# simonamtoft/downsampled-diffusion

Measured on AMD Instinct MI355X. Metric: images/sec (T=1000 sampling), 256x256 dDDPM-x3, higher is better.
Workload: dtype f32

## Files before the change

### downsampled-diffusion_amd/csrc/conv_igemm.hip

```cpp
#include <cstdlib>

#include "conv_common.h"

namespace ddk {

struct IgemmParams {
    const float* src0;
    const float* src1;
    const float* w;
    const float* bias;
    const float* resid;
    float* out;
    int c0, c1, cin;
    int B, H, W;
    int Hm, Wm;
    int Ho, Wo;
    int N, M;
    int in_stride, out_scale;
    int ntaps, nphase;
    int splits, kiters, kiters_per_split;
    long long slab_stride;
    int pre_mish, post_mish;
    float* mish_out;
    const float* dmish_src;
// ... 1093 lines not shown

int conv_init_device() {
#define HALO_ATTR(V) DDK_TRY(allow_lds(&conv3x3_halo_kernel<V>, (size_t)HALO_LDS_FLOATS * sizeof(float)));
    DDK_HALO_VARIANTS(HALO_ATTR)
#undef HALO_ATTR
#define C32_ATTR(WW)                                                                                      \
    DDK_TRY(allow_lds(&conv3x3_c32_kernel<WW, false>, (size_t)C32_LDS_BYTES));          \
    DDK_TRY(allow_lds(&conv3x3_c32_kernel<WW, true>, (size_t)C32_LDS_BYTES));
    DDK_C32_WIDTHS(C32_ATTR)
#undef C32_ATTR
#define DMA_ATTR(BM, BN, WM, WN, NS) DDK_TRY(allow_lds(&igemm_dma_kernel<BM, BN, WM, WN, NS>, dma_lds_bytes<BM, BN, WM, WN, NS>()));
    DMA_ATTR(128, 128, 2, 2, 2)
    DMA_ATTR(128, 64, 2, 2, 2) DMA_ATTR(128, 64, 2, 2, 4)
    DMA_ATTR(64, 64, 2, 2, 2) DMA_ATTR(64, 64, 2, 2, 4) DMA_ATTR(64, 64, 2, 2, 6)
    DMA_ATTR(128, 32, 4, 1, 2)
    DMA_ATTR(64, 32, 2, 1, 2)
#undef DMA_ATTR
    DDK_TRY(allow_lds(&igemm_kernel<128, 128, 2, 2>, reg_lds_bytes(128, 128)));
    DDK_TRY(allow_lds(&igemm_kernel<128, 64, 2, 2>, reg_lds_bytes(128, 64)));
    DDK_TRY(allow_lds(&igemm_kernel<64, 64, 2, 2>, reg_lds_bytes(64, 64)));
    DDK_TRY(allow_lds(&igemm_kernel<128, 32, 4, 1>, reg_lds_bytes(128, 32)));
    DDK_TRY(allow_lds(&igemm_kernel<64, 32, 2, 1>, reg_lds_bytes(64, 32)));
    return DDK_OK;
}

size_t conv_workspace_bytes(int kind, int B, int H, int W, int cin, int N) {
    Geometry g;
    if (!conv_geometry(kind, H, W, g) || cin <= 0 || cin % 32) return 0;
    const Choice c = plan_conv(kind, B, H, W, cin, N, g).c;
    size_t need = c.splits == 1 ? 0 : (size_t)c.splits * B * g.Ho * g.Wo * N * sizeof(float);
    if (kind == DDK_CONVT4X4_S2 && convT_wino_ok(H, W, cin, N)) {
        const int s = convT_wino_splits(B, H, W, cin, N);
        const size_t w = s == 1 ? 0 : (size_t)s * B * g.Ho * g.Wo * N * sizeof(float);
        if (w > need) need = w;
    }
    return need;
}

bool conv_ln_fold_ok(int B, int H, int W, int cin, int N) {
    const bool off = tuning_flag("DDK_NO_LN_FOLD");
    Geometry g;
    if (off || !conv_geometry(DDK_CONV1X1, H, W, g) || cin <= 0 || cin % 32 || N % 32) return false;
    const Choice c = choose_tile((long long)B * H * W, N, 1, cin / 32);
    return c.splits == 1 && (c.tile == T64x64 || c.tile == T128x64 || c.tile == T128x128);
}

int conv_forward(const ddk_conv_args& a, hipStream_t st, const ConvLnFold* ln, const WinoGnFuse* fuse) {
    Geometry g;
    DDK_REQUIRE(conv_geometry(a.kind, a.H, a.W, g), "conv kind");
    DDK_REQUIRE(a.src0 && a.out, "conv: null src0/out");
    DDK_REQUIRE(a.weight || a.weight_wino, "conv: null weight");
    DDK_REQUIRE(a.c0 > 0 && a.c0 % 32 == 0, "conv: c0 must be a positive multiple of 32");
    DDK_REQUIRE((a.src1 == nullptr) == (a.c1 == 0), "conv: src1/c1 mismatch");
    DDK_REQUIRE(a.c1 % 32 == 0, "conv: c1 must be a multiple of 32");
    DDK_REQUIRE(a.N > 0 && a.N % 32 == 0, "conv: N must be a positive multiple of 32");
    DDK_REQUIRE(a.B > 0 && a.H > 0 && a.W > 0, "conv: B/H/W");
    DDK_REQUIRE(aligned16(a.src0) && aligned16(a.src1) && aligned16(a.weight) && aligned16(a.out) &&
                    aligned16(a.bias) && aligned16(a.resid),
                "conv: pointers must be 16-byte aligned");
    DDK_REQUIRE((long long)a.B * g.Ho * g.Wo * a.N < (1LL << 31) && (long long)a.B * a.H * a.W * (a.c0 + a.c1) < (1LL << 31),
                "conv: tensor too large for 32-bit pixel indexing");

#ifdef DDK_HOST_SANITIZE
    {
        const long long pix_in = (long long)a.B * a.H * a.W, pix_out = (long long)a.B * g.Ho * g.Wo;
        san::extent("conv src0", a.src0, pix_in * a.c0 * 4);
        san::extent("conv src1", a.src1, pix_in * a.c1 * 4);
        if (!a.defer_reduce) san::extent("conv out", a.out, pix_out * a.N * 4);
        san::extent("conv resid", a.resid, pix_out * a.N * 4);
        san::extent("conv bias", a.bias, (long long)a.N * 4);
        san::extent("conv workspace", a.workspace, (long long)a.workspace_bytes);
        san::extent("conv mish_out", a.mish_out, pix_out * a.N * 4);
        san::extent("conv dmish_src", a.dmish_src, pix_out * a.N * 4);
        if (a.gn_partials && a.gn_groups > 0) san::extent("conv gn_partials", a.gn_partials, (pix_out / 128) * a.gn_groups * 8);
    }
#endif
    DDK_REQUIRE(aligned16(a.mish_out) && aligned16(a.dmish_src), "conv: mish_out / dmish_src alignment");
    DDK_REQUIRE(!(a.mish_out || a.dmish_src) || !(a.defer_reduce || a.gn_partials || fuse || ln),
                "conv: mish_out / dmish_src go with a plain conv (no deferred reduce, GroupNorm partials or LayerNorm folding)");
    const bool act_epilogue = a.mish_out || a.dmish_src;
    if (a.weight_wino && !a.pre_mish && !act_epilogue && conv_wino_ok(a.kind, a.H, a.W, a.c0 + a.c1, a.N)) {
        DDK_REQUIRE(aligned16(a.weight_wino), "conv: weight_wino alignment");
        DDK_TRY(ensure_device_init());
        const int ws = conv_wino_splits(a.B, a.H, a.W, a.c0 + a.c1, a.N);
        const long long slab = (long long)a.B * a.H * a.W * a.N;
        if (ws > 1) {
            const size_t need = (size_t)(fuse ? ws - 1 : ws) * slab * sizeof(float);
            if (!a.workspace || a.workspace_bytes < need) {
                set_error("conv(wino): split-K workspace too small (%zu < %zu)", a.workspace_bytes, need);
                return DDK_ERR_WORKSPACE;
            }
            DDK_REQUIRE(aligned16(a.workspace), "conv: workspace alignment");
        }
        DDK_REQUIRE((long long)a.B * a.H * a.W * (a.c0 > a.c1 ? a.c0 : a.c1) * 4 < (1LL << 31), "conv(wino): a source of 2 GiB or more");
        DDK_TRY(conv_wino_forward(a, ws, st, fuse));
        if (ws > 1 && !a.defer_reduce && !fuse) {
            const long long n4 = slab / 4;
            const int blocks = (int)(ceil_div(n4, 256) < 2048 ? ceil_div(n4, 256) : 2048);
            hipLaunchKernelGGL(splitk_reduce_kernel, dim3(blocks), dim3(256), 0, st, static_cast<const float*>(a.workspace), ws, slab, a.bias,
                               a.resid, a.out, n4, a.N, a.post_mish, static_cast<float*>(nullptr), static_cast<const float*>(nullptr));
            DDK_TRY(check_launch("splitk_reduce_kernel"));
        }
        return DDK_OK;
    }
    if (a.kind == DDK_CONVT4X4_S2 && a.weight_wino && a.c1 == 0 && !a.pre_mish && !a.post_mish && !a.resid && !act_epilogue && !a.gn_partials &&
        !fuse && !ln && convT_wino_ok(a.H, a.W, a.c0, a.N)) {
        DDK_REQUIRE(aligned16(a.weight_wino), "conv: weight_wino alignment");
        DDK_TRY(ensure_device_init());
        const int ws = convT_wino_splits(a.B, a.H, a.W, a.c0, a.N);
        const long long slab = (long long)a.B * g.Ho * g.Wo * a.N;
        if (ws > 1) {
            const size_t need = (size_t)(fuse ? ws - 1 : ws) * slab * sizeof(float);
            if (!a.workspace || a.workspace_bytes < need) {
                set_error("conv(winoT): split-K workspace too small (%zu < %zu)", a.workspace_bytes, need);
                return DDK_ERR_WORKSPACE;
            }
            DDK_REQUIRE(aligned16(a.workspace), "conv: workspace alignment");
        }
        DDK_REQUIRE((long long)a.B * a.H * a.W * a.c0 * 4 < (1LL << 31), "conv(winoT): a source of 2 GiB or more");
        DDK_TRY(convT_wino_forward(a, ws, st));
        if (ws > 1 && !a.defer_reduce && !fuse) {
            const long long n4 = slab / 4;
            const int blocks = (int)(ceil_div(n4, 256) < 2048 ? ceil_div(n4, 256) : 2048);
            hipLaunchKernelGGL(splitk_reduce_kernel, dim3(blocks), dim3(256), 0, st, static_cast<const float*>(a.workspace), ws, slab, a.bias,
                               a.resid, a.out, n4, a.N, a.post_mish, static_cast<float*>(nullptr), static_cast<const float*>(nullptr));
            DDK_TRY(check_launch("splitk_reduce_kernel"));
        }
        return DDK_OK;
    }
    DDK_REQUIRE(a.weight, "conv: weight is null and the shape / arguments do not take the Winograd path (ddk_conv_wino_splits() == 0, "
                          "pre_mish, mish_out or dmish_src)");
    if (a.kind == DDK_CONV1X1 && a.c1 == 0 && !a.pre_mish && !a.post_mish && !a.defer_reduce && !a.gn_partials && !fuse && !act_epilogue &&
        !tuning_flag("DDK_NO_CONV1X1_WS") && conv1x1_ws_ok((long long)a.B * a.H * a.W, a.c0, a.N) &&
        ((long long)a.B * a.H * a.W / 64) * (a.N / 128) >= 256 &&
        (!ln || ((long long)a.B * a.H * a.W / 64) * (a.N / 128) >= 16 * 256 ||
         (256 % (a.N / 128) == 0 && ((long long)a.B * a.H * a.W / 64) % (256 / (a.N / 128)) == 0))) {
        return conv1x1_ws(a.src0, a.weight, a.bias, a.resid, a.out, (long long)a.B * a.H * a.W, a.N, ln, st);
    }
    if (a.kind == DDK_CONV1X1 && !a.pre_mish && !a.post_mish && !a.defer_reduce && !a.gn_partials && !fuse && !act_epilogue &&
        !tuning_flag("DDK_NO_CONV1X1_SM") && conv1x1_sm_ok((long long)a.B * a.H * a.W, a.c0, a.c1, a.N) &&
        (!ln || (a.c1 == 0 && ((long long)a.B * a.H * a.W / 32) * (a.N / 32) <= 512)))
        return conv1x1_sm(a.src0, a.c0, a.src1, a.c1, a.weight, a.bias, a.resid, a.out, (long long)a.B * a.H * a.W, a.N, ln, st);
    if (a.kind == DDK_CONV1X1 && a.c1 == 0 && !a.defer_reduce && !a.gn_partials && !fuse && !ln && !tuning_flag("DDK_NO_CONV1X1_STREAM") &&
        conv1x1_stream_ok((long long)a.B * a.H * a.W, a.c0, a.N))
        return conv1x1_stream(a.src0, a.c0, a.weight, a.bias, a.dmish_src, a.resid, a.out, a.mish_out, (long long)a.B * a.H * a.W, a.N,
                              a.pre_mish, a.post_mish, st);
    DDK_REQUIRE(!a.gn_partials, "conv: gn_partials is only produced by the Winograd path (weight_wino given, ddk_conv_gn_partials() > 0)");
    DDK_REQUIRE(!fuse, "conv: the in-launch GroupNorm exists on the Winograd path only");
    IgemmParams p{};
    p.src0 = a.src0; p.src1 = a.src1; p.w = a.weight; p.bias = a.bias; p.resid = a.resid; p.out = a.out;
    p.c0 = a.c0; p.c1 = a.c1; p.cin = a.c0 + a.c1;
    p.B = a.B; p.H = a.H; p.W = a.W;
    p.Hm = g.Hm; p.Wm = g.Wm; p.Ho = g.Ho; p.Wo = g.Wo;
    p.N = a.N; p.M = a.B * g.Hm * g.Wm;
    p.in_stride = g.in_stride; p.out_scale = g.out_scale;
    p.ntaps = g.ntaps; p.nphase = g.nphase;
    p.kiters = g.ntaps * (p.cin / 32);
    p.pre_mish = a.pre_mish;
    p.debug = tuning_int("DDK_DEBUG", 0);
    p.post_mish = a.post_mish;
    p.mish_out = a.mish_out; p.dmish_src = a.dmish_src;
    p.slab_stride = (long long)a.B * g.Ho * g.Wo * a.N;
    p.dWm = make_fastdiv_u((unsigned)g.Wm);
    p.dHm = make_fastdiv_u((unsigned)g.Hm);
    p.tapmode = (a.kind == DDK_CONV1X1) ? 0 : (a.kind == DDK_CONVT4X4_S2 ? 2 : (a.kind == DDK_CONV4X4_S2 ? 3 : 1));
    if (!ln && !a.defer_reduce && choose_c32(a.kind, a.B, a.H, a.W, p.cin, p.N, a.c1, a.pre_mish != 0)) {
        const int TR = 128 / a.W, TB = TR > a.H ? TR / a.H : 1, rows_img = TB > 1 ? a.H : TR;
// ... 92 lines not shown
```

### downsampled-diffusion_amd/csrc/conv_wino.hip

```cpp
#include <atomic>
#include <cstdlib>
#include <type_traits>
#include <utility>

#include "cluster_sync.h"
#include "conv_common.h"
#include "pack_elems.h"

namespace ddk {

__device__ __attribute__((aligned(128))) float g_wino_zero[32];

struct WinoParams {
    const float* src0;
    const float* src1;
    const float* wu;
    const float* bias;
    const float* resid;
    float* out;
    int c0, c1, cin;
    int B, H, W, TH, TW;
    int N, tiles;
    int splits, chunks, chunks_per_split;
    long long slab_stride;
// ... 483 lines not shown
    const long long mt = ceil_div((long long)B * (H / 2) * (W / 2), WBT);
    return (N % 128 == 0 && mt * (N / 128) >= 224) ? WINO_V_F : WINO_V_D;
}
static int wino_nt(int variant) { return variant == WINO_V_F ? 128 : WBN; }
bool conv_wino_ok(int kind, int H, int W, int cin, int N) {
    return kind == DDK_CONV3X3_S1 && H >= 2 && W >= 2 && H % 2 == 0 && W % 2 == 0 && cin > 0 && cin % 32 == 0 && N % 64 == 0;
}

int conv_wino_splits(int B, int H, int W, int cin, int N) {
    const long long tiles = (long long)B * (H / 2) * (W / 2);
    const long long wgs = ceil_div(tiles, WBT) * (N / wino_nt(wino_variant(B, H, W, N)));
    const int chunks = cin / 32;
    int s = 1;
    while (wgs * s < 256 && s * 2 <= chunks) s *= 2;
    const int cps = (int)ceil_div(chunks, s);
    return (int)ceil_div(chunks, cps);
}

static int wino_stats_shape_parts(int B, int H, int W, int cin, int N, int groups) {
    if (!conv_wino_ok(DDK_CONV3X3_S1, H, W, cin, N) || groups <= 0 || N % groups) return 0;
    const int cpg = N / groups, tpi = (H / 2) * (W / 2), nt_w = wino_nt(wino_variant(B, H, W, N));
    if (cpg % 4 || nt_w % cpg || nt_w / cpg > 8 || tpi % WBT || tpi / WBT > 32) return 0;
    return tpi / WBT;
}
int conv_wino_stats_parts(int B, int H, int W, int cin, int N, int groups) {
    if (conv_wino_splits(B, H, W, cin, N) != 1) return 0;
    return wino_stats_shape_parts(B, H, W, cin, N, groups);
}

bool convT_wino_ok(int H, int W, int cin, int N) {
    return H >= 2 && W >= 2 && H % 2 == 0 && W % 2 == 0 && cin > 0 && cin % 32 == 0 && N > 0 && N % WT_NT == 0;
}
int convT_wino_splits(int B, int H, int W, int cin, int N) {
    const long long wgs = ceil_div((long long)B * (H / 2) * (W / 2), WBT) * (N / WT_NT) * 4;
    const int chunks = cin / 32;
    int s = 1;
    while (wgs * s < 256 && s * 2 <= chunks) s *= 2;
    const int cps = (int)ceil_div(chunks, s);
    return (int)ceil_div(chunks, cps);
}
int convT_wino_forward(const ddk_conv_args& a, int splits, hipStream_t st) {
    WinoParams p{};
    p.src0 = a.src0; p.wu = a.weight_wino; p.bias = a.bias; p.out = a.out;
    p.c0 = a.c0; p.c1 = 0; p.cin = a.c0;
    p.B = a.B; p.H = a.H; p.W = a.W; p.TH = a.H / 2; p.TW = a.W / 2;
    p.N = a.N; p.tiles = a.B * p.TH * p.TW;
    p.chunks = p.cin / 32;
    p.chunks_per_split = (int)ceil_div(p.chunks, splits);
    p.splits = (int)ceil_div(p.chunks, p.chunks_per_split);
    p.slab_stride = (long long)a.B * (2 * a.H) * (2 * a.W) * a.N;
    p.dTW = make_fastdiv_u((unsigned)p.TW);
    p.dTH = make_fastdiv_u((unsigned)p.TH);
    if (p.splits > 1) p.out = static_cast<float*>(a.workspace);
    dim3 grid((unsigned)ceil_div(p.tiles, WBT), (unsigned)(a.N / WT_NT), (unsigned)(4 * p.splits));
#ifdef DDK_TUNING
    if (getenv("DDK_WINO_STAMPS")) {
        hipLaunchKernelGGL(convT_wino_kernel<1>, grid, dim3(1024), WT_LDS_FL * sizeof(float), st, p);
        return check_launch("convT_wino_kernel<dbg>");
    }
#endif
    hipLaunchKernelGGL(convT_wino_kernel<0>, grid, dim3(1024), WT_LDS_FL * sizeof(float), st, p);
    return check_launch("convT_wino_kernel");
}

int conv_wino_init_device() {
    DDK_HIP(hipFuncSetAttribute(reinterpret_cast<const void*>(&convT_wino_kernel<0>), hipFuncAttributeMaxDynamicSharedMemorySize,
                                (int)(WT_LDS_FL * sizeof(float))));
#ifdef DDK_TUNING
    DDK_HIP(hipFuncSetAttribute(reinterpret_cast<const void*>(&convT_wino_kernel<1>), hipFuncAttributeMaxDynamicSharedMemorySize,
                                (int)(WT_LDS_FL * sizeof(float))));
#endif
    DDK_HIP(hipFuncSetAttribute(reinterpret_cast<const void*>(&conv3x3_wino_kernel<0>), hipFuncAttributeMaxDynamicSharedMemorySize,
                                (int)(W_LDS_FLOATS * sizeof(float))));
    DDK_HIP(hipFuncSetAttribute(reinterpret_cast<const void*>(&conv3x3_wino_kernel<0, true>), hipFuncAttributeMaxDynamicSharedMemorySize,
                                (int)(W_LDS_FLOATS * sizeof(float))));
    DDK_HIP(hipFuncSetAttribute(reinterpret_cast<const void*>(&conv3x3_wino2_kernel<2, 0, false>), hipFuncAttributeMaxDynamicSharedMemorySize,
                                (int)(W2<2>::LDS_FL * sizeof(float))));
    DDK_HIP(hipFuncSetAttribute(reinterpret_cast<const void*>(&conv3x3_wino2_kernel<2, 0, true>), hipFuncAttributeMaxDynamicSharedMemorySize,
                                (int)(W2<2>::LDS_FL * sizeof(float))));
    DDK_HIP(hipFuncSetAttribute(reinterpret_cast<const void*>(&conv3x3_wino2_kernel<4, 0, false>), hipFuncAttributeMaxDynamicSharedMemorySize,
                                (int)(W2<4>::LDS_FL * sizeof(float))));
    DDK_HIP(hipFuncSetAttribute(reinterpret_cast<const void*>(&conv3x3_wino2_kernel<4, 0, true>), hipFuncAttributeMaxDynamicSharedMemorySize,
                                (int)(W2<4>::LDS_FL * sizeof(float))));
#ifdef DDK_TUNING
#define W2_DBG_ATTR(P_, D_) DDK_HIP(hipFuncSetAttribute(reinterpret_cast<const void*>(&conv3x3_wino2_kernel<P_, D_, false>), \
                                                hipFuncAttributeMaxDynamicSharedMemorySize, (int)(W2<P_>::LDS_FL * sizeof(float))))
    W2_DBG_ATTR(2, 1); W2_DBG_ATTR(2, 7); W2_DBG_ATTR(2, 9); W2_DBG_ATTR(2, 15); W2_DBG_ATTR(2, 17);
    W2_DBG_ATTR(4, 1); W2_DBG_ATTR(4, 7); W2_DBG_ATTR(4, 9); W2_DBG_ATTR(4, 15); W2_DBG_ATTR(4, 17);
#undef W2_DBG_ATTR
    DDK_HIP(hipFuncSetAttribute(reinterpret_cast<const void*>(&conv3x3_wino_kernel<1>), hipFuncAttributeMaxDynamicSharedMemorySize, (int)(W_LDS_FLOATS * sizeof(float))));
    DDK_HIP(hipFuncSetAttribute(reinterpret_cast<const void*>(&conv3x3_wino_kernel<2>), hipFuncAttributeMaxDynamicSharedMemorySize, (int)(W_LDS_FLOATS * sizeof(float))));
    DDK_HIP(hipFuncSetAttribute(reinterpret_cast<const void*>(&conv3x3_wino_kernel<3>), hipFuncAttributeMaxDynamicSharedMemorySize, (int)(W_LDS_FLOATS * sizeof(float))));
    DDK_HIP(hipFuncSetAttribute(reinterpret_cast<const void*>(&conv3x3_wino_kernel<4>), hipFuncAttributeMaxDynamicSharedMemorySize, (int)(W_LDS_FLOATS * sizeof(float))));
#endif
    return DDK_OK;
}

int conv_wino_cluster_np(int B, int H, int W, int cin, int N, int groups) {
    const int np = conv_wino_stats_parts(B, H, W, cin, N, groups);
    if (np <= 0 || np > 8) return 0;
    const int nt_w = wino_nt(wino_variant(B, H, W, N));
    if (N / groups > 32 || nt_w % (N / groups)) return 0;
    if (nt_w / (N / groups) > 8) return 0;
    const long long mt = (long long)B * np, nt = N / nt_w;
    if ((mt * nt) % 8) return 0;
    const long long run = mt * nt / 8;
    const long long per_round = run < 32 ? run : 32;
    if (run % (np * nt) || per_round % (np * nt)) return 0;
    return np;
}
int conv_wino_cluster_split_np(int B, int H, int W, int cin, int N, int groups, int* splits_out) {
    if (!conv_wino_ok(DDK_CONV3X3_S1, H, W, cin, N)) return 0;
    const int splits = conv_wino_splits(B, H, W, cin, N);
    if (splits_out) *splits_out = splits;
    if (splits <= 1 || splits > 4) return 0;
    const int np = wino_stats_shape_parts(B, H, W, cin, N, groups);
    if (np <= 0 || np > 8) return 0;
    const int variant = wino_variant(B, H, W, N);
    if (variant != WINO_V_D) return 0;
    const int nt_w = wino_nt(variant);
    if (N / groups > 32 || nt_w % (N / groups) || nt_w / (N / groups) > 8) return 0;
    const long long mt = (long long)B * np, nt = N / nt_w;
    if (mt * nt * splits > 256) return 0;
    return np;
}
size_t conv_wino_cluster_pair_words(int B, int H, int W, int N) {
    return (size_t)ceil_div((long long)B * (H / 2) * (W / 2), WBT) * (size_t)(N / WBN) * 16;
}
size_t conv_wino_cluster_ws_floats(int B, int H, int W, int N) {
    const long long mt = (long long)B * (H / 2) * (W / 2) / WBT, nt = N / WBN;
    return (size_t)(mt * nt * 32 + (long long)B * nt * 16);
}

bool conv_wino_cluster_device_ok() {
    static std::atomic<int> cached[64];
    int dev = 0;
    if (hipGetDevice(&dev) != hipSuccess || dev < 0 || dev >= 64) return false;
    int v = cached[dev].load(std::memory_order_relaxed);
    if (v == 0) {
        int cus = 0, xccs = 0;
        bool ok = hipDeviceGetAttribute(&cus, hipDeviceAttributeMultiprocessorCount, dev) == hipSuccess && cus == 256;
        ok = ok && hipDeviceGetAttribute(&xccs, hipDeviceAttributeNumberOfXccs, dev) == hipSuccess && xccs == 8;
        ok = ok && !getenv("HSA_CU_MASK") && !getenv("ROC_GLOBAL_CU_MASK");
        (void)hipGetLastError();
        v = ok ? 1 : 2;
        cached[dev].store(v, std::memory_order_relaxed);
    }
    return v == 1;
}

bool conv_wino_variant_new(int B, int H, int W, int N) { return wino_variant(B, H, W, N) != WINO_V_OLD; }

int conv_wino_forward(const ddk_conv_args& a, int splits, hipStream_t st, const WinoGnFuse* fuse) {
    WinoParams p{};
    if (fuse) {
        const int np = splits == 1 ? conv_wino_cluster_np(a.B, a.H, a.W, a.c0 + a.c1, a.N, fuse->groups)
                                   : conv_wino_cluster_split_np(a.B, a.H, a.W, a.c0 + a.c1, a.N, fuse->groups, nullptr);
        DDK_REQUIRE(np > 0 && !a.post_mish && !a.gn_partials, "conv(wino): shape not eligible for the in-launch GroupNorm");
        if (splits > 1) {
            DDK_REQUIRE(fuse->pairs && a.workspace && aligned16(a.workspace) && !fuse->res_x,
                        "conv(wino, cluster): a split shape needs pair counters and the slab workspace");
            p.cl_slab = static_cast<float*>(a.workspace);
            p.cl_pair = fuse->pairs;
        }
        DDK_REQUIRE(fuse->gamma && fuse->beta && fuse->records && fuse->counters && aligned16(fuse->gamma) && aligned16(fuse->beta) &&
                        aligned16(fuse->temb) && fuse->temb_stride % 4 == 0 && aligned16(fuse->records) && aligned16(fuse->counters),
                    "conv(wino): in-launch GroupNorm arguments");
        p.gn_gamma = fuse->gamma; p.gn_beta = fuse->beta; p.gn_temb = fuse->temb; p.gn_temb_rows = fuse->temb_rows;
        p.gn_temb_stride = fuse->temb_stride; p.gn_eps = fuse->eps;
        p.cl_rec = fuse->records; p.cl_cnt = fuse->counters; p.cl_fail = fuse->fail; p.cl_np = np;
        if (fuse->res_x) {
            DDK_REQUIRE(fuse->res_w && fuse->res_cin > 0 && fuse->res_cin <= 8 && fuse->res_ld >= fuse->res_cin && !a.resid,
                        "conv(wino, cluster): the 1x1 addend takes <= 8 input channels and excludes a tensor addend");
            DDK_REQUIRE(wino_variant(a.B, a.H, a.W, a.N) != WINO_V_OLD, "conv(wino, cluster): the 1x1 addend exists in the 8-matrix-wave kernels only");
            p.r1_x = fuse->res_x; p.r1_w = fuse->res_w; p.r1_b = fuse->res_b; p.r1_cin = fuse->res_cin; p.r1_ld = fuse->res_ld;
        }
        p.groups = fuse->groups;
        p.cpg = a.N / fuse->groups;
    }
    if (a.gn_partials) {
        DDK_REQUIRE(conv_wino_stats_parts(a.B, a.H, a.W, a.c0 + a.c1, a.N, a.gn_groups) > 0 && splits == 1 && !a.resid && !a.post_mish,
                    "conv: gn_partials needs a shape with ddk_conv_gn_partials() > 0 and no resid / post_mish");
        DDK_REQUIRE((reinterpret_cast<uintptr_t>(a.gn_partials) & 7u) == 0, "conv: gn_partials alignment");
        p.gn_part = reinterpret_cast<float2*>(a.gn_partials);
        p.groups = a.gn_groups;
        p.cpg = a.N / a.gn_groups;
    }
    p.src0 = a.src0; p.src1 = a.src1; p.wu = a.weight_wino; p.bias = a.bias; p.resid = a.resid; p.out = a.out;
    p.c0 = a.c0; p.c1 = a.c1; p.cin = a.c0 + a.c1;
    p.B = a.B; p.H = a.H; p.W = a.W; p.TH = a.H / 2; p.TW = a.W / 2;
    p.N = a.N; p.tiles = a.B * p.TH * p.TW;
    p.chunks = p.cin / 32;
    p.chunks_per_split = (int)ceil_div(p.chunks, splits);
    p.splits = (int)ceil_div(p.chunks, p.chunks_per_split);
    p.slab_stride = (long long)a.B * a.H * a.W * a.N;
    p.post_mish = a.post_mish;
    p.dTW = make_fastdiv_u((unsigned)p.TW);
    p.dTH = make_fastdiv_u((unsigned)p.TH);
    if (p.splits > 1 && !fuse) p.out = static_cast<float*>(a.workspace);
    const int variant = wino_variant(a.B, a.H, a.W, a.N);
    if (variant != WINO_V_OLD) {
        dim3 grid2((unsigned)ceil_div(p.tiles, WBT), (unsigned)(a.N / wino_nt(variant)), (unsigned)p.splits);
        const bool f = variant == WINO_V_F;
        const size_t lds = (size_t)(f ? W2<2>::LDS_FL : W2<4>::LDS_FL) * sizeof(float);
#ifdef DDK_TUNING
        if (getenv("DDK_WINO_STAMPS")) {
            const int v = getenv("DDK_WINO_DEBUG") ? atoi(getenv("DDK_WINO_DEBUG")) : 1;
#define W2_DBG_LAUNCH(D_)                                                                                              \
    if (v == D_) {                                                                                                     \
        if (f) hipLaunchKernelGGL((conv3x3_wino2_kernel<2, D_, false>), grid2, dim3(768), lds, st, p);                 \
        else hipLaunchKernelGGL((conv3x3_wino2_kernel<4, D_, false>), grid2, dim3(768), lds, st, p);                   \
        return check_launch("conv3x3_wino2_kernel<dbg>");                                                              \
    }
            W2_DBG_LAUNCH(7) W2_DBG_LAUNCH(9) W2_DBG_LAUNCH(15) W2_DBG_LAUNCH(17)
#undef W2_DBG_LAUNCH
            if (f) hipLaunchKernelGGL((conv3x3_wino2_kernel<2, 1, false>), grid2, dim3(768), lds, st, p);
            else hipLaunchKernelGGL((conv3x3_wino2_kernel<4, 1, false>), grid2, dim3(768), lds, st, p);
            return check_launch("conv3x3_wino2_kernel<dbg>");
        }
#endif
        if (fuse) {
            if (f) hipLaunchKernelGGL((conv3x3_wino2_kernel<2, 0, true>), grid2, dim3(768), lds, st, p);
            else hipLaunchKernelGGL((conv3x3_wino2_kernel<4, 0, true>), grid2, dim3(768), lds, st, p);
            return check_launch("conv3x3_wino2_kernel<cluster>");
        }
        if (f) hipLaunchKernelGGL((conv3x3_wino2_kernel<2, 0, false>), grid2, dim3(768), lds, st, p);
        else hipLaunchKernelGGL((conv3x3_wino2_kernel<4, 0, false>), grid2, dim3(768), lds, st, p);
        return check_launch("conv3x3_wino2_kernel");
    }
    dim3 grid((unsigned)ceil_div(p.tiles, WBT), (unsigned)(a.N / WBN), (unsigned)p.splits);
#ifdef DDK_TUNING
    if (getenv("DDK_WINO_STAMPS")) {
        const int v = getenv("DDK_WINO_DEBUG") ? atoi(getenv("DDK_WINO_DEBUG")) : 1;
        if (v == 2) hipLaunchKernelGGL(conv3x3_wino_kernel<2>, grid, dim3(512), W_LDS_FLOATS * sizeof(float), st, p);
        else if (v == 3) hipLaunchKernelGGL(conv3x3_wino_kernel<3>, grid, dim3(512), W_LDS_FLOATS * sizeof(float), st, p);
        else if (v == 4) hipLaunchKernelGGL(conv3x3_wino_kernel<4>, grid, dim3(512), W_LDS_FLOATS * sizeof(float), st, p);
        else hipLaunchKernelGGL(conv3x3_wino_kernel<1>, grid, dim3(512), W_LDS_FLOATS * sizeof(float), st, p);
        return check_launch("conv3x3_wino_kernel<dbg>");
    }
#endif
    if (fuse) {
        hipLaunchKernelGGL((conv3x3_wino_kernel<0, true>), grid, dim3(512), W_LDS_FLOATS * sizeof(float), st, p);
        return check_launch("conv3x3_wino_kernel<cluster>");
    }
    hipLaunchKernelGGL(conv3x3_wino_kernel<0>, grid, dim3(512), W_LDS_FLOATS * sizeof(float), st, p);
    return check_launch("conv3x3_wino_kernel");
}

__global__ __launch_bounds__(256) void occupy_kernel(unsigned long long ticks, unsigned* sink) {
    extern __shared__ float occupy_lds[];
    occupy_lds[threadIdx.x] = (float)threadIdx.x;
    __syncthreads();
    const unsigned long long t_begin = __builtin_amdgcn_s_memrealtime();
    while (__builtin_amdgcn_s_memrealtime() - t_begin < ticks) __builtin_amdgcn_s_sleep(32);
    if (occupy_lds[(threadIdx.x + 1) & 255] < 0.f && sink) *sink = 1;
}

unsigned conv_wino_cluster_timeouts() { return cl_timeouts_read(); }

int cluster_fail_check(unsigned* word, hipStream_t st, const char* who, const char* tail) {
    unsigned v = 0;
    DDK_HIP(hipMemcpyAsync(&v, word, sizeof(v), hipMemcpyDeviceToHost, st));
    DDK_HIP(hipStreamSynchronize(st));
    if (v == 0) return DDK_OK;
    DDK_HIP(hipMemsetAsync(word, 0, sizeof(v), st));
    set_error("%s: %u workgroup(s) gave up waiting for their cluster%s", who, v, tail);
    return DDK_ERR_CLUSTER;
}

}

extern "C" int ddk_pack_conv_weight_wino(const float* w_oihw, float* dst, int O, int I, int i_pad, ddk_stream_t s) {
    using namespace ddk;
    DDK_REQUIRE(w_oihw && dst && O > 0 && I > 0 && i_pad >= I && i_pad % 32 == 0, "pack_conv_weight_wino: arguments (i_pad % 32 == 0)");
    const long long total = (long long)O * i_pad;
    DDK_REQUIRE(total < (1LL << 31), "pack_conv_weight_wino: 2^31 (n, c) pairs or more");
    const long long blocks = ceil_div(total, 256);
    hipLaunchKernelGGL(pack_conv_weight_wino_kernel<false>, dim3((unsigned)(blocks < 4096 ? blocks : 4096)), dim3(256), 0, as_stream(s), w_oihw,
                       dst, O, I, i_pad, total, 0, I);
    return check_launch("pack_conv_weight_wino_kernel");
}

extern "C" int ddk_pack_convT_weight_wino(const float* w_iohw, float* dst, int I, int O, int i_pad, ddk_stream_t s) {
    using namespace ddk;
    DDK_REQUIRE(w_iohw && dst && O > 0 && I > 0 && i_pad >= I && i_pad % 32 == 0, "pack_convT_weight_wino: arguments (i_pad % 32 == 0)");
    const long long total = (long long)O * i_pad;
    const long long blocks = ceil_div(total, 256);
    hipLaunchKernelGGL(pack_convT_weight_wino_kernel, dim3((unsigned)(blocks < 4096 ? blocks : 4096)), dim3(256), 0, as_stream(s), w_iohw, dst,
                       I, O, i_pad, total);
    return check_launch("pack_convT_weight_wino_kernel");
}
extern "C" int ddk_convT_wino_splits(int B, int H, int W, int cin, int N) {
    if (!ddk::convT_wino_ok(H, W, cin, N)) return 0;
    return ddk::convT_wino_splits(B, H, W, cin, N);
}

extern "C" int ddk_pack_conv_weight_wino_dgrad(const float* w_oihw, float* dst, int O, int I, int c_lo, int c_hi, int o_pad, ddk_stream_t s) {
    using namespace ddk;
    DDK_REQUIRE(w_oihw && dst && O > 0 && I > 0 && c_lo >= 0 && c_hi > c_lo && c_hi <= I && o_pad >= O && o_pad % 32 == 0,
                "pack_conv_weight_wino_dgrad: arguments (0 <= c_lo < c_hi <= I, o_pad % 32 == 0)");
    const long long total = (long long)(c_hi - c_lo) * o_pad;
    DDK_REQUIRE(total < (1LL << 31), "pack_conv_weight_wino_dgrad: 2^31 (n, c) pairs or more");
    const long long blocks = ceil_div(total, 256);
    hipLaunchKernelGGL(pack_conv_weight_wino_kernel<true>, dim3((unsigned)(blocks < 4096 ? blocks : 4096)), dim3(256), 0, as_stream(s), w_oihw,
                       dst, c_hi - c_lo, O, o_pad, total, c_lo, I);
    return check_launch("pack_conv_weight_wino_kernel<dgrad>");
}

#ifdef DDK_TUNING
extern "C" int ddk_debug_read_wino_timeline(unsigned long long* host_out) {
    if (hipDeviceSynchronize() != hipSuccess) return -2;
    return hipMemcpyFromSymbol(host_out, HIP_SYMBOL(ddk::g_wino_timeline), sizeof(unsigned long long) * 12 * 8 * 2) == hipSuccess ? 0 : -2;
}
extern "C" int ddk_debug_read_wino_stamps(unsigned long long* host_out) {
    if (hipDeviceSynchronize() != hipSuccess) return -2;
    if (hipMemcpyFromSymbol(host_out, HIP_SYMBOL(ddk::g_wino_stamps), sizeof(unsigned long long) * 8 * 1024) != hipSuccess) return -2;
    static unsigned long long zeros[8 * 1024];
    return hipMemcpyToSymbol(HIP_SYMBOL(ddk::g_wino_stamps), zeros, sizeof(zeros)) == hipSuccess ? 0 : -2;
}
#endif

extern "C" int ddk_conv_gn_partials(int B, int H, int W, int cin, int N, int groups) {
    return ddk::conv_wino_stats_parts(B, H, W, cin, N, groups);
}

extern "C" int ddk_conv_wino_splits(int B, int H, int W, int cin, int N) {
    if (!ddk::conv_wino_ok(DDK_CONV3X3_S1, H, W, cin, N)) return 0;
    return ddk::conv_wino_splits(B, H, W, cin, N);
}

extern "C" int ddk_conv3x3_gn_mish_cluster_ok(int B, int H, int W, int cin, int N, int groups) {
    if (!ddk::conv_wino_cluster_device_ok()) return 0;
    const int np = ddk::conv_wino_cluster_np(B, H, W, cin, N, groups);
    return np > 0 ? np : ddk::conv_wino_cluster_split_np(B, H, W, cin, N, groups, nullptr);
}
extern "C" size_t ddk_conv3x3_gn_mish_cluster_workspace_bytes(int B, int H, int W, int N) {
    if (B <= 0 || H <= 0 || W <= 0 || N <= 0 || N % ddk::WBN) return 0;
    return (ddk::cl_front_floats(B) + ddk::conv_wino_cluster_ws_floats(B, H, W, N)) * sizeof(float);
}
extern "C" size_t ddk_conv3x3_gn_mish_cluster_split_workspace_bytes(int B, int H, int W, int cin, int N, int groups) {
    int splits = 1;
    if (ddk::conv_wino_cluster_split_np(B, H, W, cin, N, groups, &splits) <= 0) return 0;
    return ddk_conv3x3_gn_mish_cluster_workspace_bytes(B, H, W, N) +
           (ddk::conv_wino_cluster_pair_words(B, H, W, N) + (size_t)(splits - 1) * B * H * W * N) * sizeof(float);
}
extern "C" int ddk_conv3x3_gn_mish_cluster_check(void* workspace, int B, ddk_stream_t s) {
    using namespace ddk;
    DDK_REQUIRE(workspace && B > 0, "conv3x3_gn_mish_cluster_check: arguments");
    return cluster_fail_check(cl_words(static_cast<float*>(workspace), B).fail, as_stream(s), "conv3x3_gn_mish_cluster",
                              "; the output is invalid (NaN tiles)");
}

extern "C" int ddk_debug_occupy(int workgroups, int lds_bytes, int microseconds, ddk_stream_t s) {
    using namespace ddk;
    DDK_REQUIRE(workgroups > 0 && workgroups <= 4096 && lds_bytes >= 1024 && lds_bytes <= 160 * 1024 && microseconds > 0 &&
                    microseconds <= 200000, "debug_occupy: 1..4096 workgroups, 1 KiB..160 KiB of LDS, at most 0.2 s");
    DDK_HIP(hipFuncSetAttribute(reinterpret_cast<const void*>(&occupy_kernel), hipFuncAttributeMaxDynamicSharedMemorySize, lds_bytes));
    hipLaunchKernelGGL(occupy_kernel, dim3((unsigned)workgroups), dim3(256), (size_t)lds_bytes, as_stream(s),
                       (unsigned long long)microseconds * 100ull, static_cast<unsigned*>(nullptr));
    return check_launch("occupy_kernel");
}

extern "C" int ddk_conv3x3_gn_mish_cluster(const float* src0, int c0, const float* src1, int c1, const float* weight_wino, const float* bias,
                                           const float* gamma, const float* beta, const float* temb, int temb_stride, const float* addend,
                                           float* out, int B, int H, int W, int N, int groups, float eps, void* workspace,
                                           size_t workspace_bytes, ddk_stream_t s) {
    using namespace ddk;
    DDK_REQUIRE(src0 && weight_wino && gamma && beta && out && workspace, "conv3x3_gn_mish_cluster: null pointer");
    DDK_REQUIRE(conv_wino_cluster_device_ok() && ddk_conv3x3_gn_mish_cluster_ok(B, H, W, c0 + c1, N, groups) > 0,
                "conv3x3_gn_mish_cluster: shape or device not eligible (ddk_conv3x3_gn_mish_cluster_ok)");
    const size_t plain_bytes = ddk_conv3x3_gn_mish_cluster_workspace_bytes(B, H, W, N);
    const size_t split_bytes = ddk_conv3x3_gn_mish_cluster_split_workspace_bytes(B, H, W, c0 + c1, N, groups);
    DDK_REQUIRE(workspace_bytes >= (split_bytes ? split_bytes : plain_bytes) && aligned16(workspace), "conv3x3_gn_mish_cluster: workspace");
    float* ws = static_cast<float*>(workspace);
    DDK_HIP(hipMemsetAsync(ws, 0, cl_front_floats(B) * sizeof(float), as_stream(s)));
    float* pairs = ws + plain_bytes / sizeof(float);
    if (split_bytes) DDK_HIP(hipMemsetAsync(pairs, 0, conv_wino_cluster_pair_words(B, H, W, N) * sizeof(float), as_stream(s)));
    ddk_conv_args a{};
    a.kind = DDK_CONV3X3_S1;
    a.src0 = src0; a.src1 = src1; a.c0 = c0; a.c1 = c1;
    a.weight = weight_wino;
    a.weight_wino = weight_wino;
    a.bias = bias;
    a.resid = addend;
    a.out = out;
    a.B = B; a.H = H; a.W = W; a.N = N;
    const ClWords w = cl_words(ws, B);
    WinoGnFuse f{gamma, beta, temb, nullptr, temb_stride, eps, groups, ws + cl_front_floats(B), w.counters, w.fail};
    if (split_bytes) {
        f.pairs = reinterpret_cast<unsigned*>(pairs);
        a.workspace = pairs + conv_wino_cluster_pair_words(B, H, W, N);
        a.workspace_bytes = split_bytes - plain_bytes - conv_wino_cluster_pair_words(B, H, W, N) * sizeof(float);
    }
    return conv_forward(a, as_stream(s), nullptr, &f);
}
```

### downsampled-diffusion_amd/csrc/conv_wino2_kernel.inc

```

template <int... I, class F>
__device__ __forceinline__ void static_for_impl(std::integer_sequence<int, I...>, F&& f) { (f(std::integral_constant<int, I>{}), ...); }
template <int N, class F>
__device__ __forceinline__ void static_for(F&& f) { static_for_impl(std::make_integer_sequence<int, N>{}, f); }

#ifndef DDK_WINO2_LP_F
#define DDK_WINO2_LP_F 8
#endif
#ifndef DDK_WINO2_LP_D
#define DDK_WINO2_LP_D 4
#endif
template <int P>
struct W2 {
    static constexpr int NT = 256 / P;
    static constexpr int NB = NT / 32;
    static constexpr int SPC = 16 / P;
    static constexpr int SPR = 4 / P;
    static constexpr int V_FL = P * WBT * 32;
    static constexpr int U_FL = P * NT * 32;
    static constexpr int STAGE = V_FL + U_FL;
    static constexpr int PPI = NT / 8;
    static constexpr int TP = NT + 4;
    static constexpr int T_FL = 4 * 2 * WBT * TP;
    static constexpr int LDS_FL = (3 * STAGE > T_FL + 320) ? 3 * STAGE : T_FL + 320;
    static constexpr int QUADS = NT / 4;
    static constexpr int ITEMS = 2 * WBT * QUADS / 512;
    static constexpr int LPL = P == 2 ? DDK_WINO2_LP_F : DDK_WINO2_LP_D;
    static constexpr int LPM = (32 - 4 * LPL) / 8;
    static_assert(4 * LPL + 8 * LPM == 32 && LPL % 2 == 0 && LPM % 2 == 0, "piece split: (8,0), (4,2) or (0,4)");
};
#ifndef DDK_WINO2_STAGGER
#define DDK_WINO2_STAGGER 1
#endif
constexpr bool W2_STAGGER = DDK_WINO2_STAGGER != 0;

__device__ unsigned long long g_wino_timeline[12 * 8 * 2];

template <int P, int DBG, bool CL>
__global__ __launch_bounds__(768) void conv3x3_wino2_kernel(const WinoParams p) {
    using G = W2<P>;
    constexpr int NT = G::NT, SPC = G::SPC, SPR = G::SPR, STAGE = G::STAGE, V_FL = G::V_FL;
    extern __shared__ __attribute__((aligned(16))) float smem[];
    unsigned long long r_entry = 0;
    if (DBG) r_entry = __builtin_amdgcn_s_memrealtime();
    const int tid = threadIdx.x, lane = tid & 63;
    const int wid = __builtin_amdgcn_readfirstlane(tid >> 6);
    int tile_m, tile_n, split;
    {
        const int nwg = gridDim.x * gridDim.y * gridDim.z;
        const int bid = blockIdx.x + gridDim.x * (blockIdx.y + gridDim.y * blockIdx.z);
        const int q = nwg >> 3, r = nwg & 7, xcd = bid & 7, idx = bid >> 3;
        const int logical = (xcd < r ? xcd * (q + 1) : r * (q + 1) + (xcd - r) * q) + idx;
        tile_n = logical % gridDim.y;
        const int rest = logical / gridDim.y;
        tile_m = rest % gridDim.x;
        split = rest / gridDim.x;
    }
    const int t0 = tile_m * WBT, n0 = tile_n * NT;
    const int c_begin = split * p.chunks_per_split;
    const int n_chunks = min(p.chunks, c_begin + p.chunks_per_split) - c_begin;
    const int n_stages = n_chunks * SPC;
    const unsigned lds_base = (unsigned)(size_t)(__attribute__((address_space(3))) float*)smem;
    const int prow = lane >> 3, ppos = lane & 7;
    const unsigned uv_even = (unsigned)((prow * 32 + ((ppos ^ (prow >> 1)) << 2)) * 4);
    const unsigned uv_odd = (unsigned)((prow * 32 + ((ppos ^ (4 + (prow >> 1))) << 2)) * 4);
    auto issue_u = [&](int T, int buf, int g_first, auto count) {
        const int chunk = c_begin + T / SPC, st = T % SPC;
        const float* base = p.wu + (((long long)chunk * 16 + P * st) * p.N + n0) * 32;
        const unsigned dst = lds_base + (unsigned)((buf * STAGE + V_FL) * 4);
#pragma unroll
        for (int j = 0; j < decltype(count)::value; ++j) {
            const int g = g_first + j;
            const int image = g / G::PPI, rb = g % G::PPI;
            lds_dma16_s(base + ((long long)image * p.N + rb * 8) * 32, (j & 1) ? uv_odd : uv_even, dst + (unsigned)(g * 1024));
        }
    };

    if (wid >= 8) {
        const int lw = wid - 8;
        const int lt = lw * 64 + lane;
        const int t = lt >> 3, cq = lt & 7;
        __builtin_amdgcn_s_setprio(3);
        const int g = t0 + t;
        const bool tile_ok = g < p.tiles;
        const unsigned gg = tile_ok ? (unsigned)g : 0u;
        const unsigned tmp = fdiv_u(gg, p.dTW);
        const int tx = (int)(gg - tmp * (unsigned)p.TW);
        const unsigned bq = fdiv_u(tmp, p.dTH);
        const int ty = (int)(tmp - bq * (unsigned)p.TH), b = (int)bq;
        const int py0 = 2 * ty - 1, px0 = 2 * tx - 1;
        const int pix0 = (b * p.H + py0) * p.W + px0;
        unsigned mask = 0;
#pragma unroll
        for (int dy = 0; dy < 4; ++dy)
#pragma unroll
            for (int dx = 0; dx < 4; ++dx)
                if (tile_ok && (unsigned)(py0 + dy) < (unsigned)p.H && (unsigned)(px0 + dx) < (unsigned)p.W) mask |= 1u << (dy * 4 + dx);
        const i32x4 srd0 = make_srd(p.src0, (unsigned)((long long)p.B * p.H * p.W * p.c0 * 4));
        const i32x4 srd1 = make_srd(p.src1 ? p.src1 : p.src0, (unsigned)((long long)p.B * p.H * p.W * (p.src1 ? p.c1 : p.c0) * 4));
        unsigned voff[16];
        int cur_src = -1;
        auto set_source = [&](int which) {
            const int cs = which == 0 ? p.c0 : p.c1;
#pragma unroll
            for (int dy = 0; dy < 4; ++dy)
#pragma unroll
                for (int dx = 0; dx < 4; ++dx)
                    voff[dy * 4 + dx] = ((mask >> (dy * 4 + dx)) & 1u) ? (unsigned)(((pix0 + dy * p.W + dx) * cs + cq * 4) * 4) : WINO_OOB;
            cur_src = which;
        };
        const int v_off = t * 32 + ((cq ^ ((t >> 1) & 7)) << 2);
        f32x4 d[16];
        auto load_row = [&](int chunk, int row) {
            const int cc = chunk << 5;
            const bool first = cc < p.c0;
            if ((first ? 0 : 1) != cur_src) set_source(first ? 0 : 1);
            const unsigned soff = (unsigned)((first ? cc : cc - p.c0) * 4);
            i32x4 srd;
            srd.x = first ? srd0.x : srd1.x; srd.y = first ? srd0.y : srd1.y; srd.z = first ? srd0.z : srd1.z; srd.w = srd0.w;
#pragma unroll
            for (int dy = 0; dy < 4; ++dy)
                if (dy == row) {
#pragma unroll
                    for (int dx = 0; dx < 4; ++dx) buf_load16(d[dy * 4 + dx], voff[dy * 4 + dx], srd, soff);
                }
        };
        auto pin = [&]() {
#pragma unroll
            for (int i = 0; i < 16; ++i) asm volatile("" : "+v"(d[i]));
        };
        auto write_v = [&](auto kc, auto hc, int buf) {
            constexpr int k = decltype(kc)::value, h = decltype(hc)::value;
            auto rowc = [&](auto xc) -> f32x4 {
                constexpr int x = decltype(xc)::value;
                if constexpr (k == 0) return d[0 * 4 + x] - d[2 * 4 + x];
                else if constexpr (k == 1) return d[1 * 4 + x] + d[2 * 4 + x];
                else if constexpr (k == 2) return d[2 * 4 + x] - d[1 * 4 + x];
                else return d[1 * 4 + x] - d[3 * 4 + x];
            };
            using I0 = std::integral_constant<int, 0>; using I1 = std::integral_constant<int, 1>;
            using I2 = std::integral_constant<int, 2>; using I3 = std::integral_constant<int, 3>;
            float* base = smem + buf * STAGE + v_off;
            if constexpr (P == 4) {
                const f32x4 r0 = rowc(I0{}), r1 = rowc(I1{}), r2 = rowc(I2{}), r3 = rowc(I3{});
                *reinterpret_cast<f32x4*>(base + 0 * (WBT * 32)) = r0 - r2;
                *reinterpret_cast<f32x4*>(base + 1 * (WBT * 32)) = r1 + r2;
                *reinterpret_cast<f32x4*>(base + 2 * (WBT * 32)) = r2 - r1;
                *reinterpret_cast<f32x4*>(base + 3 * (WBT * 32)) = r1 - r3;
            } else if constexpr (h == 0) {
                const f32x4 r0 = rowc(I0{}), r1 = rowc(I1{}), r2 = rowc(I2{});
                *reinterpret_cast<f32x4*>(base + 0 * (WBT * 32)) = r0 - r2;
                *reinterpret_cast<f32x4*>(base + 1 * (WBT * 32)) = r1 + r2;
            } else {
                const f32x4 r1 = rowc(I1{}), r2 = rowc(I2{}), r3 = rowc(I3{});
                *reinterpret_cast<f32x4*>(base + 0 * (WBT * 32)) = r2 - r1;
                *reinterpret_cast<f32x4*>(base + 1 * (WBT * 32)) = r1 - r3;
            }
        };
        auto produce = [&](auto tsc, int T, int tc, int buf) -> bool {
            constexpr int ts = decltype(tsc)::value, k = ts / SPR, h = ts % SPR;
            if (!(DBG & 8)) write_v(std::integral_constant<int, k>{}, std::integral_constant<int, h>{}, buf);
            bool loaded = false;
            if constexpr (h == SPR - 1 && !(DBG & 8)) {
                if (k == 1) { load_row(c_begin + tc, 3); loaded = true; }
                else if (tc + 1 < n_chunks) { load_row(c_begin + tc + 1, k == 0 ? 0 : k == 2 ? 2 : 1); loaded = true; }
            }
            if (!(DBG & 2)) issue_u(T, buf, lw * G::LPL, std::integral_constant<int, G::LPL>{});
            return loaded;
        };
        load_row(c_begin, 0);
        load_row(c_begin, 2);
        if (P == 4) load_row(c_begin, 1);
        if (!(DBG & 2)) issue_u(0, 0, lw * G::LPL, std::integral_constant<int, G::LPL>{});
        if (P == 2) load_row(c_begin, 1);
        constexpr int NPL0 = (DBG & 2) ? 0 : G::LPL;
        wait_vmcnt<NPL0 + (P == 2 ? 4 : 0)>();
        pin();
        using K0 = std::integral_constant<int, 0>;
        if (!(DBG & 8)) {
            write_v(K0{}, K0{}, 0);
            if (P == 2) write_v(K0{}, std::integral_constant<int, SPR - 1>{}, 1);
            else write_v(std::integral_constant<int, 1 / SPR>{}, K0{}, 1);
            if (1 < n_chunks) load_row(c_begin + 1, 0);
            if (P == 4) load_row(c_begin, 3);
        }
        if (!(DBG & 2)) issue_u(1, 1, lw * G::LPL, std::integral_constant<int, G::LPL>{});
        if (DBG & 8) wait_vmcnt<NPL0>();
        else if (P == 2) { if (1 < n_chunks) wait_vmcnt<NPL0 + 8>(); else wait_vmcnt<NPL0 + 4>(); }
        else { if (1 < n_chunks) wait_vmcnt<NPL0 + 8>(); else wait_vmcnt<NPL0 + 4>(); }
        asm volatile("s_waitcnt lgkmcnt(0)" ::: "memory");
        __builtin_amdgcn_s_barrier();
        int b0 = 0;
        for (int qi = 0; qi < n_chunks; ++qi) {
            static_for<SPC>([&](auto sc) {
                constexpr int s = decltype(sc)::value;
                const int S = qi * SPC + s;
                const int buf2 = b0 == 0 ? 2 : b0 - 1;
                const bool more = S + 2 < n_stages;
                if (s == 0 && qi == 0) wait_vmcnt<((DBG & 2) ? 0 : G::LPL)>();
                pin();
                bool loaded = false;
                if (more) {
                    constexpr int ts = (s + 2) % SPC;
                    loaded = produce(std::integral_constant<int, ts>{}, S + 2, qi + (s + 2 >= SPC ? 1 : 0), buf2);
                }
                constexpr int NPL = (DBG & 2) ? 0 : G::LPL;
                if (more) { if (loaded) wait_vmcnt<NPL + 4>(); else wait_vmcnt<NPL>(); }
                else wait_vmcnt<0>();
                asm volatile("s_waitcnt lgkmcnt(0)" ::: "memory");
                unsigned long long tlA = 0;
                const bool tl = (DBG & 16) && blockIdx.x + blockIdx.y + blockIdx.z == 0 && S >= 8 && S < 16;
                if (tl) asm volatile("s_memtime %0\n\ts_waitcnt lgkmcnt(0)" : "=s"(tlA)::"memory");
                __builtin_amdgcn_s_barrier();
                if (tl) {
                    unsigned long long tlB;
                    asm volatile("s_memtime %0\n\ts_waitcnt lgkmcnt(0)" : "=s"(tlB)::"memory");
                    if (lane == 0) { g_wino_timeline[(wid * 8 + (S - 8)) * 2] = tlA; g_wino_timeline[(wid * 8 + (S - 8)) * 2 + 1] = tlB; }
                }
                b0 = b0 == 2 ? 0 : b0 + 1;
            });
        }
        return;
    }

    const int pp = wid % P, nb = wid / P;
    f32x16 acc[SPC];
#pragma unroll
    for (int i = 0; i < SPC; ++i)
#pragma unroll
        for (int r = 0; r < 16; ++r) acc[i][r] = 0.f;
    {
        const int fsw = ((lane & 31) >> 1) & 7, fh = lane >> 5;
        int foff[4];
#pragma unroll
        for (int q = 0; q < 4; ++q) foff[q] = (lane & 31) * 32 + (((2 * q + fh) ^ fsw) << 2);
        const int a_img = pp * (WBT * 32), b_img = V_FL + (pp * NT + nb * 32) * 32;
        if (G::LPM > 0 && !(DBG & 4)) {
            issue_u(0, 0, 4 * G::LPL + wid * G::LPM, std::integral_constant<int, G::LPM>{});
            issue_u(1, 1, 4 * G::LPL + wid * G::LPM, std::integral_constant<int, G::LPM>{});
            wait_vmcnt<G::LPM>();
        }
        __builtin_amdgcn_s_barrier();
        unsigned long long r_loop0 = 0, c_wait = 0, c_mma = 0;
        if (DBG) r_loop0 = __builtin_amdgcn_s_memrealtime();
        auto mloop = [&](auto stgc) {
            constexpr bool STG = decltype(stgc)::value;
            float4 a[2], b[2];
            int buf = 0, S = 0;
            auto frag = [&](float4& av, float4& bv, const float* As, const float* Bs, int q) {
                av = *reinterpret_cast<const float4*>(As + foff[q]);
                bv = *reinterpret_cast<const float4*>(Bs + foff[q]);
            };
            auto mma4 = [&](f32x16& c, const float4& av, const float4& bv) {
                c = __builtin_amdgcn_mfma_f32_32x32x2f32(av.x, bv.x, c, 0, 0, 0);
                c = __builtin_amdgcn_mfma_f32_32x32x2f32(av.y, bv.y, c, 0, 0, 0);
                c = __builtin_amdgcn_mfma_f32_32x32x2f32(av.z, bv.z, c, 0, 0, 0);
                c = __builtin_amdgcn_mfma_f32_32x32x2f32(av.w, bv.w, c, 0, 0, 0);
            };
            if (STG) frag(a[1], b[1], smem + a_img, smem + b_img, 0);
            else a[0] = *reinterpret_cast<const float4*>(smem + a_img + foff[0]);
            for (int c = 0; c < n_chunks; ++c) {
                static_for<SPC>([&](auto sc) {
                    constexpr int s = decltype(sc)::value;
                    const float* As = smem + buf * STAGE + a_img;
                    const float* Bs = smem + buf * STAGE + b_img;
                    const int nbuf = buf == 2 ? 0 : buf + 1, pbuf = buf == 0 ? 2 : buf - 1;
                    const bool more = S + 2 < n_stages;
                    auto dma = [&] {
                        if (more && G::LPM > 0 && !(DBG & 4)) {
                            __builtin_amdgcn_sched_barrier(0);
                            issue_u(S + 2, pbuf, 4 * G::LPL + wid * G::LPM, std::integral_constant<int, G::LPM>{});
                            __builtin_amdgcn_sched_barrier(0);
                        }
                    };
                    if constexpr (!STG) {
                        b[0] = *reinterpret_cast<const float4*>(Bs + foff[0]);
                        frag(a[1], b[1], As, Bs, 1);
                        __builtin_amdgcn_sched_barrier(0);
                        mma4(acc[s], a[0], b[0]);
                        frag(a[0], b[0], As, Bs, 2);
                        __builtin_amdgcn_sched_barrier(0);
                        mma4(acc[s], a[1], b[1]);
                        dma();
                        frag(a[1], b[1], As, Bs, 3);
                        __builtin_amdgcn_sched_barrier(0);
                        mma4(acc[s], a[0], b[0]);
                        a[0] = *reinterpret_cast<const float4*>(smem + nbuf * STAGE + a_img + foff[0]);
                        __builtin_amdgcn_sched_barrier(0);
                        mma4(acc[s], a[1], b[1]);
                    } else {
                        if (s > 0 || c > 0) {
                            frag(a[1], b[1], As, Bs, 0);
                            __builtin_amdgcn_sched_barrier(0);
                            mma4(acc[(s + SPC - 1) % SPC], a[0], b[0]);
                        }
                        frag(a[0], b[0], As, Bs, 1);
                        __builtin_amdgcn_sched_barrier(0);
                        mma4(acc[s], a[1], b[1]);
                        dma();
                        frag(a[1], b[1], As, Bs, 2);
                        __builtin_amdgcn_sched_barrier(0);
                        mma4(acc[s], a[0], b[0]);
                        frag(a[0], b[0], As, Bs, 3);
                        __builtin_amdgcn_sched_barrier(0);
                        mma4(acc[s], a[1], b[1]);
                    }
                    if (more && !(DBG & 4)) wait_vmcnt<G::LPM>(); else wait_vmcnt<0>();
                    unsigned long long tA = 0, tB = 0;
                    if (DBG) { asm volatile("s_memtime %0\n\ts_waitcnt lgkmcnt(0)" : "=s"(tA)::"memory"); }
                    __builtin_amdgcn_s_barrier();
                    if (DBG) { asm volatile("s_memtime %0\n\ts_waitcnt lgkmcnt(0)" : "=s"(tB)::"memory"); c_wait += tB - tA; if (c_mma == 0) c_mma = tA; }
                    if ((DBG & 16) && blockIdx.x + blockIdx.y + blockIdx.z == 0 && S >= 8 && S < 16 && lane == 0) {
                        g_wino_timeline[(wid * 8 + (S - 8)) * 2] = tA;
                        g_wino_timeline[(wid * 8 + (S - 8)) * 2 + 1] = tB;
                    }
                    buf = nbuf;
                    ++S;
                });
            }
            if (STG) mma4(acc[SPC - 1], a[0], b[0]);
        };
        if (W2_STAGGER && wid >= 4) mloop(std::true_type{}); else mloop(std::false_type{});
        if (DBG && lane == 0 && wid == 0) {
            const int wg = (blockIdx.x + gridDim.x * (blockIdx.y + gridDim.y * blockIdx.z)) & 1023;
            unsigned long long tE;
            asm volatile("s_memtime %0\n\ts_waitcnt lgkmcnt(0)" : "=s"(tE)::"memory");
            g_wino_stamps[wg * 8 + 0] = r_entry;
            g_wino_stamps[wg * 8 + 1] = r_loop0;
            g_wino_stamps[wg * 8 + 2] = __builtin_amdgcn_s_memrealtime();
            g_wino_stamps[wg * 8 + 3] = c_wait;
            g_wino_stamps[wg * 8 + 4] = tE - c_mma;
            g_wino_stamps[wg * 8 + 5] = (unsigned long long)n_stages;
        }
    }
    {
        constexpr int TP = G::TP;
#pragma unroll
        for (int r = 0; r < 16; ++r) {
            const int row = (r & 3) + 8 * (r >> 2) + 4 * (lane >> 5);
            const int col = nb * 32 + (lane & 31);
            if constexpr (P == 4) {
                float* Ts = smem + pp * (2 * WBT * TP);
                const float m0 = acc[0][r], m1 = acc[1][r], m2 = acc[2][r], m3 = acc[3][r];
                Ts[row * TP + col] = (m0 + m1) + m2;
                Ts[(WBT + row) * TP + col] = (m1 - m2) - m3;
            } else {
                const float l0 = acc[0][r], l1 = acc[2][r], l2 = acc[4][r], l3 = acc[6][r];
                const float h0 = acc[1][r], h1 = acc[3][r], h2 = acc[5][r], h3 = acc[7][r];
                const float tl0 = (l0 + l1) + l2, tl1 = (l1 - l2) - l3;
                const float th0 = (h0 + h1) + h2, th1 = (h1 - h2) - h3;
                float* B0 = smem + (pp * 2 + 0) * (2 * WBT * TP);
                float* B1 = smem + (pp * 2 + 1) * (2 * WBT * TP);
                if (pp == 0) {
                    B0[row * TP + col] = tl0 + th0;          B0[(WBT + row) * TP + col] = tl1 + th1;
                    B1[row * TP + col] = -th0;               B1[(WBT + row) * TP + col] = -th1;
                } else {
                    B0[row * TP + col] = tl0;                B0[(WBT + row) * TP + col] = tl1;
                    B1[row * TP + col] = tl0 - th0;          B1[(WBT + row) * TP + col] = tl1 - th1;
                }
            }
        }
    }
    __syncthreads();

    constexpr int TP = G::TP, QUADS = G::QUADS, ITEMS = G::ITEMS;
    constexpr bool CLS = CL && P == 4;
    const bool partner = CLS && split > 0;
    const bool direct = p.splits == 1 || (CLS && !partner);
    float* outp = p.splits == 1 ? p.out : CLS ? p.cl_slab + (long long)(split - 1) * p.slab_stride : p.out + (long long)split * p.slab_stride;
    float4 keep[ITEMS][2];
    long long oo[ITEMS];
    int opix[ITEMS];
    const int cq = tid & (QUADS - 1);
    const int gn = n0 + cq * 4;
#pragma unroll
    for (int it = 0; it < ITEMS; ++it) {
        const int item = tid + it * 512;
        const int t = item / (2 * QUADS), a = (item / QUADS) & 1;
        const int g = t0 + t;
        keep[it][0] = keep[it][1] = make_float4(0.f, 0.f, 0.f, 0.f);
        oo[it] = -1;
        opix[it] = 0;
        if (g >= p.tiles || gn >= p.N) continue;
        const float* tp = smem + (a * WBT + t) * TP + cq * 4;
        const float4 q0 = *reinterpret_cast<const float4*>(tp);
        const float4 q1 = *reinterpret_cast<const float4*>(tp + 1 * (2 * WBT * TP));
        const float4 q2 = *reinterpret_cast<const float4*>(tp + 2 * (2 * WBT * TP));
        const float4 q3 = *reinterpret_cast<const float4*>(tp + 3 * (2 * WBT * TP));
        float4 y0, y1;
        if constexpr (P == 4) {
            y0 = f4add(f4add(q0, q1), q2);
            y1 = f4sub(f4sub(q1, q2), q3);
        } else {
            y0 = f4add(q0, q2);
            y1 = f4add(q1, q3);
        }
        const unsigned tmp = fdiv_u((unsigned)g, p.dTW);
        const int tx = g - (int)tmp * p.TW;
        const unsigned bq = fdiv_u(tmp, p.dTH);
        const int ty = (int)tmp - (int)bq * p.TH;
        const long long o0 = ((((long long)bq * p.H + 2 * ty + a) * p.W) + 2 * tx) * p.N + gn;
        oo[it] = o0;
        opix[it] = ((int)bq * p.H + 2 * ty + a) * p.W + 2 * tx;
        if (direct) {
            if (p.bias) {
                const float4 bb = *reinterpret_cast<const float4*>(p.bias + gn);
                y0 = f4add(y0, bb);
                y1 = f4add(y1, bb);
            }
            if (!CL && p.resid) {
                y0 = f4add(y0, *reinterpret_cast<const float4*>(p.resid + o0));
                y1 = f4add(y1, *reinterpret_cast<const float4*>(p.resid + o0 + p.N));
            }
            if (p.post_mish) {
                y0 = make_float4(mish_f(y0.x), mish_f(y0.y), mish_f(y0.z), mish_f(y0.w));
                y1 = make_float4(mish_f(y1.x), mish_f(y1.y), mish_f(y1.z), mish_f(y1.w));
            }
        }
        if (!CL) {
            *reinterpret_cast<float4*>(outp + o0) = y0;
            *reinterpret_cast<float4*>(outp + o0 + p.N) = y1;
        } else if (CLS && partner) {
            st_sc1_f4(outp + o0, y0);
            st_sc1_f4(outp + o0 + p.N, y1);
        }
        keep[it][0] = y0;
        keep[it][1] = y1;
    }
    if (CLS && p.splits > 1) {
        unsigned* pair = p.cl_pair + ((long long)tile_m * gridDim.y + tile_n) * 16;
        if (partner) {
            asm volatile("s_waitcnt vmcnt(0)" ::: "memory");
            __syncthreads();
            if (tid == 0) __hip_atomic_fetch_add(pair, 1u, __ATOMIC_RELAXED, __HIP_MEMORY_SCOPE_AGENT);
            return;
        }
        int* pair_gave_up = reinterpret_cast<int*>(smem + G::T_FL + 258);
        if (tid == 0) {
            *pair_gave_up = 0;
            const unsigned want = (unsigned)p.splits - 1u;
            if (cl_wait_ge<2>(pair, want, p.cl_fail)) *pair_gave_up = 1;
            __hip_atomic_store(pair, 0u, __ATOMIC_RELAXED, __HIP_MEMORY_SCOPE_AGENT);
        }
        __syncthreads();
        const bool pair_poisoned = *pair_gave_up != 0;
        for (int s = 1; s < p.splits; ++s) {
            const float* sl = p.cl_slab + (long long)(s - 1) * p.slab_stride;
            static_assert(ITEMS % 2 == 0, "two items per load group");
#pragma unroll
            for (int it = 0; it < ITEMS; it += 2) {
                float4 a0, a1, b0, b1;
                ld_sc1_f4x4(a0, a1, b0, b1, sl + oo[it], sl + oo[it] + p.N, sl + oo[it + 1], sl + oo[it + 1] + p.N);
                keep[it][0] = f4add(keep[it][0], a0);
                keep[it][1] = f4add(keep[it][1], a1);
                keep[it + 1][0] = f4add(keep[it + 1][0], b0);
                keep[it + 1][1] = f4add(keep[it + 1][1], b1);
            }
        }
        if (pair_poisoned) {
#pragma unroll
            for (int it = 0; it < ITEMS; ++it) keep[it][0].x = __builtin_nanf("");
        }
    }
    if (CL || p.gn_part) {
        const int qpg = p.cpg >> 2;
        const int gl = cq / qpg;
        float* red = smem + G::T_FL;
        auto group_sum = [&](float v, float* rd) {
            for (int o = 1; o < qpg; o <<= 1) v += __shfl_xor(v, o, 64);
#pragma unroll
            for (int o = QUADS; o < 64; o <<= 1) v += __shfl_xor(v, o, 64);
            if (lane < QUADS && (cq & (qpg - 1)) == 0) rd[wid * 16 + gl] = v;
            asm volatile("s_waitcnt lgkmcnt(0)\n\ts_barrier" ::: "memory");
            float t = rd[gl];
#pragma unroll
            for (int w = 1; w < 8; ++w) t += rd[w * 16 + gl];
            return t;
        };
        auto sum4 = [](float4 v) { return (v.x + v.y) + (v.z + v.w); };
        const float inv = 1.0f / (float)(4 * WBT * p.cpg);
        float s1 = 0.f;
#pragma unroll
        for (int it = 0; it < ITEMS; ++it) s1 += sum4(keep[it][0]) + sum4(keep[it][1]);
        const float mean = group_sum(s1, red) * inv;
        auto sq4 = [&](float4 v) {
            const float a = v.x - mean, b = v.y - mean, c = v.z - mean, d = v.w - mean;
            return (a * a + b * b) + (c * c + d * d);
        };
        float s2 = 0.f;
#pragma unroll
        for (int it = 0; it < ITEMS; ++it) s2 += sq4(keep[it][0]) + sq4(keep[it][1]);
        const float m2 = group_sum(s2, red + 128);
        if (!CL) {
            if (tid < QUADS && (cq & (qpg - 1)) == 0) p.gn_part[(long long)tile_m * p.groups + n0 / p.cpg + gl] = make_float2(mean, m2);
        } else {
            const int image = tile_m / p.cl_np;
            unsigned long long* rec = reinterpret_cast<unsigned long long*>(p.cl_rec) + ((long long)tile_m * gridDim.y + tile_n) * 16;
            unsigned* cnt = p.cl_cnt + ((long long)image * gridDim.y + tile_n) * 16;
            int* gave_up = reinterpret_cast<int*>(red + 256);
            if (tid == 0) *gave_up = 0;
            if (tid < QUADS && (cq & (qpg - 1)) == 0) cl_store_stats(rec + gl, mean, m2);
            float4 ga, be, ts = make_float4(0.f, 0.f, 0.f, 0.f);
            auto load_affine = [&] {
                ga = *reinterpret_cast<const float4*>(p.gn_gamma + gn);
                be = *reinterpret_cast<const float4*>(p.gn_beta + gn);
                if (p.gn_temb) {
                    const int b_img = (int)((long long)t0 / ((long long)p.TH * p.TW));
                    const long long tr = p.gn_temb_rows ? p.gn_temb_rows[b_img] : b_img;
                    ts = *reinterpret_cast<const float4*>(p.gn_temb + tr * p.gn_temb_stride + gn);
                }
            };
            float4 rs[ITEMS][2];
// ... 87 lines not shown
```

### downsampled-diffusion_amd/csrc/ddk_internal.h

```cpp
#pragma once
#include <hip/hip_runtime.h>

#include <cstdarg>
#include <cstdint>
#include <cstdio>

#include "ddk.h"

#ifdef DDK_HOST_SANITIZE
#include "host_sanitize.h"
#endif

namespace ddk {

void set_error(const char* fmt, ...);

inline int fail_arg(const char* what) {
    set_error("bad argument: %s", what);
    return DDK_ERR_ARG;
}

inline int check_launch(const char* what) {
    hipError_t e = hipGetLastError();
    if (e != hipSuccess) {
// ... 24 lines not shown
    } while (0)

inline bool aligned16(const void* p) { return (reinterpret_cast<uintptr_t>(p) & 15u) == 0; }
inline hipStream_t as_stream(ddk_stream_t s) { return reinterpret_cast<hipStream_t>(s); }
inline long long ceil_div(long long a, long long b) { return (a + b - 1) / b; }

__device__ __forceinline__ float mish_f(float x) {
    if (x > 20.0f) return x;
    const float e = __expf(x);
    const float n = e * (e + 2.0f);
    return x * (n * __frcp_rn(n + 2.0f));
}

__device__ __forceinline__ float mish_grad_f(float u) {
    if (u > 20.0f) return 1.0f;
    const float e = __expf(u);
    const float n = e * (e + 2.0f);
    const float r = __frcp_rn(n + 2.0f);
    return n * r + u * (4.0f * e * (e + 1.0f)) * (r * r);
}

__device__ __forceinline__ int div_upr(int u, int upr) {
    return (upr & (upr - 1)) == 0 ? u >> (31 - __builtin_clz(upr)) : u / upr;
}
__device__ __forceinline__ long long div_upr(long long u, int upr) {
    return (upr & (upr - 1)) == 0 ? u >> (31 - __builtin_clz(upr)) : u / upr;
}

__device__ __forceinline__ float wave_sum(float v) {
#pragma unroll
    for (int o = 32; o > 0; o >>= 1) v += __shfl_xor(v, o, 64);
    return v;
}

__device__ __forceinline__ float wave_max(float v) {
#pragma unroll
    for (int o = 32; o > 0; o >>= 1) v = fmaxf(v, __shfl_xor(v, o, 64));
    return v;
}

__device__ __forceinline__ float block_sum(float v, float* red) {
    v = wave_sum(v);
    const int lane = threadIdx.x & 63, wid = threadIdx.x >> 6, nw = blockDim.x >> 6;
    __syncthreads();
    if (lane == 0) red[wid] = v;
    __syncthreads();
    float t = (lane < nw) ? red[lane] : 0.0f;
    t = wave_sum(t);
    return t;
}

__device__ __forceinline__ float block_max(float v, float* red) {
    v = wave_max(v);
    const int lane = threadIdx.x & 63, wid = threadIdx.x >> 6, nw = blockDim.x >> 6;
    __syncthreads();
    if (lane == 0) red[wid] = v;
    __syncthreads();
    float t = (lane < nw) ? red[lane] : -INFINITY;
    t = wave_max(t);
    return t;
}

int ensure_device_init();
int conv_init_device();
int wgrad_init_device();

size_t conv_workspace_bytes(int kind, int B, int H, int W, int cin, int N);
struct ConvLnFold {
    const float* c1;
    const float* c2;
    float eps;
};
struct WinoGnFuse {
    const float* gamma;
    const float* beta;
    const float* temb;
    const long long* temb_rows;
    int temb_stride;
    float eps;
    int groups;
    float* records;
    unsigned* counters;
    unsigned* fail;
    unsigned* pairs = nullptr;
    const float* res_x = nullptr;
    const float* res_w = nullptr;
    const float* res_b = nullptr;
    int res_cin = 0, res_ld = 0;
};
bool conv_ln_fold_ok(int B, int H, int W, int cin, int N);
int conv_forward(const ddk_conv_args& a, hipStream_t st, const ConvLnFold* ln = nullptr, const WinoGnFuse* fuse = nullptr);
int conv_splits(int kind, int B, int H, int W, int cin, int N);
bool conv_wino_ok(int kind, int H, int W, int cin, int N);
int conv_wino_splits(int B, int H, int W, int cin, int N);
int conv_wino_forward(const ddk_conv_args& a, int splits, hipStream_t st, const WinoGnFuse* fuse = nullptr);
int conv_wino_cluster_np(int B, int H, int W, int cin, int N, int groups);
int conv_wino_cluster_split_np(int B, int H, int W, int cin, int N, int groups, int* splits_out);
size_t conv_wino_cluster_pair_words(int B, int H, int W, int N);
bool conv_wino_variant_new(int B, int H, int W, int N);
bool conv_wino_cluster_device_ok();
size_t conv_wino_cluster_ws_floats(int B, int H, int W, int N);
unsigned conv_wino_cluster_timeouts();
unsigned conv_first_cluster_timeouts();
unsigned level_chain_cluster_timeouts();
constexpr size_t CL_PAIR_WORDS = 128 * 16;
inline size_t cl_fail_offset(int B) { return (size_t)B * 8 * 16; }
inline size_t cl_front_floats(int B) { return cl_fail_offset(B) + 16; }
inline size_t cl_chain_offset(int B) { return cl_front_floats(B); }
inline size_t cl_pair_offset(int B) { return cl_chain_offset(B) + (size_t)B * 64; }
inline size_t cl_counter_floats(int B) { return cl_pair_offset(B) + CL_PAIR_WORDS; }
struct ClWords { unsigned* counters; unsigned* fail; };
inline ClWords cl_words(float* cl, int B) { return {reinterpret_cast<unsigned*>(cl), reinterpret_cast<unsigned*>(cl + cl_fail_offset(B))}; }
int cluster_fail_check(unsigned* word, hipStream_t st, const char* who, const char* tail);
bool convT_wino_ok(int H, int W, int cin, int N);
int convT_wino_splits(int B, int H, int W, int cin, int N);
int convT_wino_forward(const ddk_conv_args& a, int splits, hipStream_t st);
int conv_wino_init_device();
int conv_wino_stats_parts(int B, int H, int W, int cin, int N, int groups);
bool conv_first_ok(int cin, int N, int H, int W, int groups);
int conv_first(const float* x, const float* wp, const float* bias, float* out, float* gn_partials, int B, int H, int W, int cin, int N,
               int groups, int64_t* counter, int64_t* t_cur, hipStream_t st);
int conv_first_init_device();
bool conv_first_gn_ok(int cin, int N, int H, int W, int groups);
size_t conv_first_gn_ws_floats(int B, int H, int W);
int conv_first_gn(const float* x, const float* wp, const float* bias, const float* gamma, const float* beta, const float* temb,
                  int temb_stride, const long long* temb_rows, float eps, float* out, int B, int H, int W, int cin, int N, int groups,
                  float* records, unsigned* counters, unsigned* fail, int64_t* counter, int64_t* t_cur, hipStream_t st);
bool conv1x1_sm_ok(long long M, int c0, int c1, int N);
int conv1x1_sm(const float* src0, int c0, const float* src1, int c1, const float* w, const float* bias, const float* resid, float* out,
               long long M, int N, const ConvLnFold* ln, hipStream_t st);
int conv1x1_sm_init_device();
bool conv1x1_stream_ok(long long M, int cin, int N);
int conv1x1_stream(const float* x, int cin, const float* w, const float* bias, const float* dmish_src, const float* resid, float* out,
                   float* mish_out, long long M, int N, int pre_mish, int post_mish, hipStream_t st);
bool conv1x1_ws_ok(long long M, int K, int N);
int conv1x1_ws(const float* x, const float* w, const float* bias, const float* resid, float* out, long long M, int N, const ConvLnFold* ln,
               hipStream_t st, int images = 0);
int conv1x1_ws_init_device();
struct AddendSlabs {
    int n = 1;
    long long stride = 0;
    const float* bias = nullptr;
};
bool conv_gn_local_ok(int H, int W, int cin, int c0, int N, int groups);
int conv_gn_local(const float* src0, int c0, const float* src1, int c1, const float* w, const float* bias, const float* gamma,
                  const float* beta, const float* temb, int temb_stride, const long long* temb_rows, const float* addend, float* out,
                  int B, int H, int W, int N, int groups, float eps, hipStream_t st, const AddendSlabs& as = AddendSlabs(),
                  const AddendSlabs& src_slabs = AddendSlabs());
int conv_gn_local_init_device();
bool conv_gn_wlocal_ok(int H, int W, int cin, int c0, int N, int groups);
int conv_gn_wlocal(const float* src0, int c0, const float* src1, int c1, const float* w, const float* bias, const float* gamma,
                   const float* beta, const float* temb, int temb_stride, const long long* temb_rows, const float* addend, float* out,
                   int B, int H, int W, int N, int groups, float eps, hipStream_t st, const AddendSlabs& as = AddendSlabs(),
                   const AddendSlabs& src_slabs = AddendSlabs());
double conv_flops(int kind, int B, int H, int W, int cin, int N);
size_t groupnorm_workspace_bytes(int B, int HW, int C, int groups);
int gn_train_nsplit(int HW, int cpg);
int gn_stats_partials(const float* x, float* part, int B, int HW, int C, int groups, int ns, hipStream_t st);
int groupnorm_mish(const float* x, const float* gamma, const float* beta, const float* temb, int temb_stride,
                   const float* addend, float* out, int B, int HW, int C, int groups, float eps, void* ws, size_t ws_bytes,
                   hipStream_t st, const long long* temb_rows = nullptr);
int groupnorm_mish_ex(const float* x, int nslab, long long slab_stride, const float* cbias, const float* gamma,
                      const float* beta, const float* temb, int temb_stride, const float* addend, float* out, int B, int HW, int C,
                      int groups, float eps, void* ws, size_t ws_bytes, hipStream_t st, const long long* temb_rows = nullptr);
int groupnorm_mish_parts(const float* x, const float* part, int np, const float* gamma, const float* beta, const float* temb,
                         int temb_stride, const float* addend, float* out, int B, int HW, int C, int groups, float eps, hipStream_t st,
                         const long long* temb_rows = nullptr, const float* rc_x = nullptr, const float* rc_w = nullptr,
                         const float* rc_b = nullptr, int rc_cin = 0, int rc_ld = 0);
int chan_layernorm(const float* x, const float* g, const float* b, float* out, long long M, int C, float eps, hipStream_t st);
int groupnorm_mish_generic(const float* x, const float* gamma, const float* beta, const float* temb, int temb_stride, const float* addend,
                           float* out, int B, int HW, int CP, int C, int groups, float eps, hipStream_t st, const long long* temb_rows = nullptr);
int chan_layernorm_generic(const float* x, const float* g, const float* b, float* out, long long M, int CP, int C, float eps, hipStream_t st);
int unary(int op, const float* x, float* out, long long n, hipStream_t st);
int add(const float* a, const float* b, float* out, long long n, hipStream_t st);
int avgpool2(const float* x, float* out, int B, int H, int W, int C, hipStream_t st);
int upsample_nearest2(const float* x, float* out, int B, int H, int W, int C, hipStream_t st);
size_t linattn_context_workspace_bytes(int B, int HW, int heads);
int linattn_context(const float* qkv, float* ctx, int B, int HW, int heads, void* workspace, size_t workspace_bytes, hipStream_t st,
                    bool kv_only = false);
bool attn_fold_ok(int C, int heads);
// ... 101 lines not shown
```

### downsampled-diffusion_amd/csrc/unet_plan.hip

```cpp
#include <algorithm>
#include <mutex>
#include <string>
#include <vector>

#include "ddk_internal.h"
#include "level_chain.h"

namespace ddk {

constexpr int HEADS = 4;
constexpr int HIDDEN = HEADS * 32;
constexpr int GROUPS = 8;
constexpr float GN_EPS = 1e-5f, LN_EPS = 1e-5f;

static inline int pad32(int c) { return (c + 31) / 32 * 32; }

enum PackKind { PK_COPY = 0, PK_CONV = 1, PK_CONVT = 2, PK_LINEAR_T = 3, PK_WINO = 4, PK_LOCAL = 5, PK_WLOCAL = 6, PK_FIRST = 7, PK_CONVT_WINO = 8,
                PK_ROWS = 9 , PK_LOCAL1 = 10 ,
                PK_CONVT_LOCAL = 11  };

struct Slot {
    std::string name;
    long long numel;
    int kind;
// ... 7 lines not shown
    size_t w = 0, b = 0;
    bool has_bias = false;
    int cin = 0, cin_pad = 0, cout = 0;
    size_t wu = 0;
    bool has_wu = false;
    size_t wl = 0;
    bool has_wl = false;
    size_t wwl = 0;
    bool has_wwl = false;
    size_t wf = 0;
    bool has_wf = false;
    size_t wl1 = 0;
    bool has_wl1 = false;
    size_t wtl = 0;
    bool has_wtl = false;
};
struct NormW { size_t g = 0, b = 0; int c_real = 0; };
struct ResW {
    int ci = 0, ci_pad = 0, co = 0, temb_off = 0, ci_real = 0, co_real = 0;
    ConvW c1, c2, res;
    NormW n1, n2;
    bool has_res = false;
};
struct AttnW {
    int c = 0, c_real = 0;
    NormW ln;
    ConvW qkv, out;
    size_t qkv_lnw = 0, ln_c1 = 0, ln_c2 = 0;
    size_t qkv_op = 0;
};

}

using namespace ddk;

struct ChainKey {
    StepKind kind;
    const void* bufs[12];
    const void* ws;
    const void* noise;
    int B, H, W, t_start, device;
    unsigned long long pack_epoch;
    int restore_n = 0;
    bool operator==(const ChainKey& o) const {
        for (int i = 0; i < 12; ++i)
            if (bufs[i] != o.bufs[i]) return false;
        return kind == o.kind && ws == o.ws && noise == o.noise && B == o.B && H == o.H && W == o.W && t_start == o.t_start &&
               device == o.device && pack_epoch == o.pack_epoch && restore_n == o.restore_n;
    }
};
struct SamplerGraph {
    ChainKey key;
    hipGraph_t graph = nullptr;
    hipGraphExec_t exec = nullptr;
    hipGraph_t graph_multi = nullptr;
    hipGraphExec_t exec_multi = nullptr;
    hipEvent_t done = nullptr;
    unsigned long long last_use = 0;
};
constexpr int SAMPLER_MULTI = 16;

struct ddk_unet {
    std::mutex mu;
    std::vector<SamplerGraph> graphs;
    unsigned long long use_clock = 0;
    unsigned long long pack_epoch = 0;
    struct {
        const void* ws = nullptr;
        int t_start = -1, B = 0, H = 0, W = 0;
        unsigned long long pack_epoch = 0;
        std::vector<int64_t> map;
    } table;
    ddk_unet_config cfg;
    int cluster_gn = 1;
    int cluster_limit = 1 << 30;
    int cluster_np_max = 8;
    bool cluster_split = true;
    bool attn_kvctx = true;
    bool fold_down_reduce = false;
    bool restore_fused = true;
    bool first_gn = true;
    int level_chain = 9;
    int level_chain_max_batch = 32;
    int attn_fold_min_hw = 256;
    bool attn_fold = true;
    bool generic = false;
    std::vector<int> dimp;
    std::vector<Slot> slots;
    size_t packed_floats = 0;
    int L = 0;
    std::vector<int> dims;
    int time_dim = 0, temb_total = 0;
    size_t freqs = 0, w1t = 0, b1 = 0, w2t = 0, b2 = 0, temb_wt = 0, temb_bias = 0;
    std::vector<ResW> down_res, up_res;
    std::vector<AttnW> down_attn, up_attn;
    std::vector<ConvW> down_conv, up_conv;
    ResW mid1, mid2;
    AttnW mid_attn;
    ConvW final_conv;
    NormW final_norm;
    size_t final_w = 0, final_b = 0;

    size_t alloc(size_t n) {
        const size_t o = packed_floats;
        packed_floats += (n + 3) / 4 * 4;
        return o;
    }
    size_t add_copy(const std::string& name, long long n) {
        const size_t o = alloc((size_t)n);
        slots.push_back(Slot{name, n, PK_COPY, o, 0, 0, 0, 0, 0, 0, 0});
        return o;
    }
    void add_copy_at(const std::string& name, long long n, size_t off) {
        slots.push_back(Slot{name, n, PK_COPY, off, 0, 0, 0, 0, 0, 0, 0});
    }
    ConvW add_conv(const std::string& prefix, int cout, int cin, int k, bool bias, bool gn_follows = false, int split = 0, bool local = false) {
        ConvW c;
        c.cin = cin; c.cin_pad = split > 0 ? pad32(split) + pad32(cin - split) : pad32(cin); c.cout = cout;
        const int cout_rows = pad32(cout);
        c.w = alloc((size_t)cout_rows * k * k * c.cin_pad);
        Slot sl{prefix + "weight", (long long)cout * cin * k * k, PK_CONV, c.w, cout, cin, k, k, c.cin_pad, 0, 0};
        if (split > 0 && c.cin_pad != cin) { sl.split = split; sl.split_pad = pad32(split); }
        slots.push_back(sl);
        c.has_bias = bias;
        if (bias) {
            c.b = alloc((size_t)cout_rows);
            slots.push_back(Slot{prefix + "bias", cout, PK_COPY, c.b, 0, 0, 0, 0, 0, 0, 0});
        }
        if (generic) return c;
        if (k == 1 && bias && cout % 32 == 0 && c.cin_pad == cin && cin % 32 == 0) {
            c.wl1 = alloc((size_t)cout * c.cin_pad);
            c.has_wl1 = true;
            slots.push_back(Slot{prefix + "weight", (long long)cout * cin, PK_LOCAL1, c.wl1, cout, cin, 1, 1, c.cin_pad, 0, 0});
        }
        if (k == 3 && cout % 64 == 0) {
            c.wu = alloc((size_t)16 * cout * c.cin_pad);
            c.has_wu = true;
            slots.push_back(Slot{prefix + "weight", (long long)cout * cin * k * k, PK_WINO, c.wu, cout, cin, k, k, c.cin_pad, 0, 0});
        }
        if (k == 3 && (gn_follows || local) && cout % 32 == 0) {
            c.wl = alloc((size_t)9 * cout * c.cin_pad);
            c.has_wl = true;
            slots.push_back(Slot{prefix + "weight", (long long)cout * cin * k * k, PK_LOCAL, c.wl, cout, cin, k, k, c.cin_pad, 0, 0});
            if (gn_follows && (c.cin_pad <= 320 || c.cin_pad == 512)) {
                c.wwl = alloc((size_t)16 * cout * c.cin_pad);
                c.has_wwl = true;
                slots.push_back(Slot{prefix + "weight", (long long)cout * cin * k * k, PK_WLOCAL, c.wwl, cout, cin, k, k, c.cin_pad, 0, 0});
            }
        }
        return c;
    }
    ConvW add_convT(const std::string& prefix, int ch, bool local = false) {
        ConvW c;
        c.cin = ch; c.cin_pad = pad32(ch); c.cout = ch;
        c.w = alloc((size_t)16 * pad32(ch) * pad32(ch));
        slots.push_back(Slot{prefix + "weight", (long long)16 * ch * ch, PK_CONVT, c.w, ch, ch, 4, 4, pad32(ch), 0, 0});
        c.has_bias = true;
        c.b = alloc((size_t)pad32(ch));
        slots.push_back(Slot{prefix + "bias", ch, PK_COPY, c.b, 0, 0, 0, 0, 0, 0, 0});
        if (local && ch % 32 == 0 && !generic) {
            c.wtl = alloc((size_t)16 * ch * ch);
            c.has_wtl = true;
            slots.push_back(Slot{prefix + "weight", (long long)16 * ch * ch, PK_CONVT_LOCAL, c.wtl, ch, ch, 4, 4, ch, 0, 0});
        }
        if (ch % 128 == 0) {
            c.wu = alloc((size_t)36 * ch * ch);
// ... 137 lines not shown
                                pad32(cfg->chan), 0});
    } else {
        u->final_w = u->add_copy("final_conv.1.weight", (long long)cfg->in_ch * cfg->chan);
    }
    u->final_b = u->add_copy("final_conv.1.bias", cfg->in_ch);
    if (cur != u->temb_total) {
        set_error("unet_create: internal temb accounting mismatch");
        delete u;
        return nullptr;
    }
    return u;
}

static void drop_graphs(ddk_unet* u) {
    for (SamplerGraph& g : u->graphs) {
        if (g.exec) (void)hipGraphExecDestroy(g.exec);
        if (g.graph) (void)hipGraphDestroy(g.graph);
        if (g.exec_multi) (void)hipGraphExecDestroy(g.exec_multi);
        if (g.graph_multi) (void)hipGraphDestroy(g.graph_multi);
        if (g.done) (void)hipEventDestroy(g.done);
    }
    u->graphs.clear();
    u->table.ws = nullptr;
}

extern "C" void ddk_unet_destroy(ddk_unet* u) {
    if (!u) return;
    if (!u->graphs.empty()) (void)hipDeviceSynchronize();
    drop_graphs(u);
    delete u;
}

extern "C" int ddk_sampler_invalidate(ddk_unet* u) {
    DDK_REQUIRE(u, "sampler_invalidate: null plan");
    std::lock_guard<std::mutex> lock(u->mu);
    if (!u->graphs.empty()) DDK_HIP(hipDeviceSynchronize());
    drop_graphs(u);
    return DDK_OK;
}
static void destroy_entry(SamplerGraph& g) {
    if (g.done) { (void)hipEventSynchronize(g.done); (void)hipEventDestroy(g.done); }
    if (g.exec) (void)hipGraphExecDestroy(g.exec);
    if (g.graph) (void)hipGraphDestroy(g.graph);
    if (g.exec_multi) (void)hipGraphExecDestroy(g.exec_multi);
    if (g.graph_multi) (void)hipGraphDestroy(g.graph_multi);
}

extern "C" int ddk_sampler_release_workspace(ddk_unet* u, const void* workspace) {
    DDK_REQUIRE(u && workspace, "sampler_release_workspace: arguments");
    std::lock_guard<std::mutex> lock(u->mu);
    for (size_t i = 0; i < u->graphs.size();) {
        if (u->graphs[i].key.ws == workspace) {
            destroy_entry(u->graphs[i]);
            u->graphs.erase(u->graphs.begin() + (long)i);
        } else {
            ++i;
        }
    }
    if (u->table.ws == workspace) u->table.ws = nullptr;
    return DDK_OK;
}

extern "C" int ddk_unet_set_option(ddk_unet* u, int option, int value) {
    DDK_REQUIRE(u, "unet_set_option: null plan");
    static const struct {
        int option;
        bool drops_graphs;
        void (*set)(ddk_unet&, int);
    } options[] = {
        {DDK_OPT_CLUSTER_GROUPNORM, true, [](ddk_unet& p, int v) { p.cluster_gn = v < 0 ? 0 : v > 2 ? 2 : v; }},
        {DDK_OPT_ATTENTION_FOLD, true, [](ddk_unet& p, int v) { p.attn_fold = v != 0; }},
        {DDK_OPT_ATTENTION_KV_CONTEXT, true, [](ddk_unet& p, int v) { p.attn_kvctx = v != 0; }},
        {DDK_OPT_FIRST_GROUPNORM, true, [](ddk_unet& p, int v) { p.first_gn = v != 0; }},
        {DDK_OPT_RESTORE_FUSED_TAIL, true, [](ddk_unet& p, int v) { p.restore_fused = v != 0; }},
        {DDK_OPT_LEVEL_CHAIN, true, [](ddk_unet& p, int v) {
             p.level_chain = v == 1 ? 9 : v == 2 ? 1 : v == 3 ? 15 : v == 4 ? 6 : v == 8 ? 2 : v == 16 ? 4 : v != 0 ? 9 : 0;
         }},
        {DDK_OPT_FOLD_DOWNSAMPLE_REDUCE, true, [](ddk_unet& p, int v) { p.fold_down_reduce = v != 0; }},
        {10, true, [](ddk_unet& p, int v) { p.level_chain_max_batch = v; }},
        {9, true, [](ddk_unet& p, int v) { p.attn_fold_min_hw = v; }},
        {2, false, [](ddk_unet& p, int v) { p.cluster_limit = v; }},
        {4, true, [](ddk_unet& p, int v) { p.cluster_np_max = v; }},
        {11, true, [](ddk_unet& p, int v) { p.cluster_split = v != 0; }},
    };
    for (const auto& o : options) {
        if (o.option != option) continue;
        std::lock_guard<std::mutex> lock(u->mu);
        if (o.drops_graphs) {
            if (!u->graphs.empty()) DDK_HIP(hipDeviceSynchronize());
            drop_graphs(u);
        }
        o.set(*u, value);
        return DDK_OK;
    }
    return fail_arg("unet_set_option: unknown option");
}
extern "C" unsigned ddk_debug_cluster_timeouts(void) {
    unsigned sum = 0;
    for (unsigned v : {ddk::conv_wino_cluster_timeouts(), ddk::conv_first_cluster_timeouts(), ddk::level_chain_cluster_timeouts()}) {
        if (v == ~0u) return ~0u;
        sum += v;
    }
    return sum;
}
extern "C" int ddk_unet_num_slots(const ddk_unet* u) { return u ? (int)u->slots.size() : 0; }
extern "C" const char* ddk_unet_slot_name(const ddk_unet* u, int slot) {
    return (u && slot >= 0 && slot < (int)u->slots.size()) ? u->slots[slot].name.c_str() : nullptr;
}
extern "C" long long ddk_unet_slot_numel(const ddk_unet* u, int slot) {
    return (u && slot >= 0 && slot < (int)u->slots.size()) ? u->slots[slot].numel : -1;
}
extern "C" size_t ddk_unet_packed_bytes(const ddk_unet* u) { return u ? u->packed_floats * sizeof(float) : 0; }

__global__ __launch_bounds__(64) void ln_fold_kernel(const float* __restrict__ w, const float* __restrict__ g, const float* __restrict__ b,
                                                     float* __restrict__ wg, float* __restrict__ c1, float* __restrict__ c2, int C, int cp) {
    const int n = blockIdx.x;
    float s1 = 0.f, s2 = 0.f;
    for (int c = threadIdx.x; c < cp; c += 64) {
        const float wv = w[(long long)n * cp + c];
        const float gv = c < C ? g[c] : 0.f, bv = c < C ? b[c] : 0.f;
        wg[(long long)n * cp + c] = wv * gv;
        s1 += wv * gv;
        s2 += wv * bv;
    }
    s1 = wave_sum(s1);
    s2 = wave_sum(s2);
    if (threadIdx.x == 0) { c1[n] = s1; c2[n] = s2; }
}

static int fold_attn(const AttnW& a, float* P, hipStream_t st) {
    hipLaunchKernelGGL(ln_fold_kernel, dim3(3 * HIDDEN), dim3(64), 0, st, P + a.qkv.w, P + a.ln.g, P + a.ln.b, P + a.qkv_lnw, P + a.ln_c1,
                       P + a.ln_c2, a.c, pad32(a.c));
    DDK_TRY(check_launch("ln_fold_kernel"));
    return qkv_operand_pack(P + a.qkv_lnw, P + a.qkv_op, HEADS, pad32(a.c), st);
}

static void weights_changed(const ddk_unet* u) {
    ddk_unet* m = const_cast<ddk_unet*>(u);
    std::lock_guard<std::mutex> lock(m->mu);
    ++m->pack_epoch;
}

extern "C" int ddk_unet_finalize_pack(const ddk_unet* u, void* packed, ddk_stream_t s) {
    DDK_REQUIRE(u && packed, "unet_finalize_pack: arguments");
    weights_changed(u);
    for (const AttnW& a : u->attn_all) DDK_TRY(fold_attn(a, static_cast<float*>(packed), as_stream(s)));
    return DDK_OK;
}

extern "C" int ddk_unet_pack_slot(const ddk_unet* u, int slot, const float* canonical, void* packed, ddk_stream_t s) {
    DDK_REQUIRE(u && canonical && packed && slot >= 0 && slot < (int)u->slots.size(), "unet_pack_slot: arguments");
    const Slot& sl = u->slots[slot];
    float* dst = static_cast<float*>(packed) + sl.off;
    weights_changed(u);
    int rc;
    switch (sl.kind) {
        case PK_COPY:
            DDK_HIP(hipMemcpyAsync(dst, canonical, (size_t)sl.numel * sizeof(float), hipMemcpyDeviceToDevice, as_stream(s)));
            rc = DDK_OK;
            break;
        case PK_CONV:
            rc = sl.split > 0 ? ddk_pack_conv_weight_split(canonical, dst, sl.O, sl.I, sl.KH, sl.KW, sl.i_pad, sl.split, sl.split_pad, s)
                              : ddk_pack_conv_weight(canonical, dst, sl.O, sl.I, sl.KH, sl.KW, sl.i_pad, s);
            break;
        case PK_CONVT: rc = sl.i_pad == sl.I ? ddk_pack_convT_weight(canonical, dst, sl.I, sl.O, s)
                                             : ddk_pack_convT_weight_padded(canonical, dst, sl.I, sl.O, sl.i_pad, s); break;
// ... 135 lines not shown
    ly.tact = al4((size_t)B * u.time_dim);
    ly.act = al4(ly.act); ly.qkv = al4(ly.qkv); ly.o = al4(ly.o); ly.ctx = al4(ly.ctx);
    ly.splitk = al4(ly.splitk); ly.gn_ws = al4(ly.gn_ws); ly.cl = al4(ly.cl);
    if (level_chain_shape_ok(u, H0, W0)) ly.chain = (size_t)CHAIN_BUFS * B * 16 * 256;
    if (level8_chain_shape_ok(u, H0, W0)) upd(ly.chain, (size_t)CHAIN8_BUFS * B * 64 * 256);

    size_t off = 0;
    auto take = [&](size_t n) { const size_t o = off; off += n; return o; };
    ly.off_A = take(ly.act); ly.off_B = take(ly.act); ly.off_C = take(ly.act);
    ly.off_raw = take(ly.act); ly.off_a1 = take(ly.act); ly.off_res = take(ly.act); ly.off_xn = take(ly.act);
    ly.off_qkv = take(ly.qkv); ly.off_o = take(ly.o); ly.off_ctx = take(ly.ctx);
    ly.off_splitk = take(ly.splitk); ly.off_gn = take(ly.gn_ws); ly.off_cl = take(ly.cl); ly.off_chain = take(ly.chain);
    ly.off_xpad = take(ly.xpad); ly.off_temb = take(ly.temb); ly.off_tact = take(ly.tact);
    ly.off_skip.resize(u.L);
    for (int l = 0; l < u.L; ++l) ly.off_skip[l] = take(ly.skip[l]);
    ly.total = off;
    return ly;
}

struct Ctx {
    const ddk_unet& u;
    const float* P;
    float* W;
    const Layout& ly;
    int B;
    hipStream_t st;
    const float* temb;
    const long long* temb_rows;
    bool allow_cluster = false;
    int n_cluster = 0;
    const float* x_first = nullptr;
    const float* x_padded = nullptr;

    ddk_conv_args conv_args(int kind, const ConvW& cw, const float* src0, int c0, const float* src1, int c1, float* out, int H, int Wd, int N,
                            const float* weight_override = nullptr) const {
        ddk_conv_args a{};
        a.kind = kind;
        a.src0 = src0; a.src1 = src1; a.c0 = c0; a.c1 = c1;
        a.weight = weight_override ? weight_override : P + cw.w;
        a.bias = cw.has_bias ? P + cw.b : nullptr;
        a.out = out;
        a.B = B; a.H = H; a.W = Wd; a.N = N;
        a.workspace = W + ly.off_splitk;
        a.workspace_bytes = ly.splitk * sizeof(float);
        if (kind == DDK_CONV3X3_S1 && !weight_override && use_wino(cw, H, Wd, c0 + c1, N)) a.weight_wino = P + cw.wu;
        if (kind == DDK_CONVT4X4_S2 && !weight_override && cw.has_wu && !src1 && convT_wino_use(B, H, Wd, c0, N)) a.weight_wino = P + cw.wu;
        return a;
    }
    WinoGnFuse gn_fuse(const NormW& n, const float* temb_shift, const long long* rows) const {
        float* cl = W + ly.off_cl;
        const ClWords w = cl_words(cl, B);
        return WinoGnFuse{P + n.g, P + n.b, temb_shift, rows, u.temb_total, GN_EPS, GROUPS, cl + cl_counter_floats(B), w.counters, w.fail};
    }
};

static int run_conv(Ctx& c, int kind, const ConvW& cw, const float* src0, int c0, const float* src1, int c1, const float* resid,
                    float* out, int H, int W, int N, const float* weight_override = nullptr, const ConvLnFold* ln = nullptr) {
    ddk_conv_args a = c.conv_args(kind, cw, src0, c0, src1, c1, out, H, W, N, weight_override);
    a.resid = resid;
    return conv_forward(a, c.st, ln);
}
static int run_conv_slabs(Ctx& c, int kind, const ConvW& cw, const float* src0, int c0, const float* src1, int c1, float* out, int H, int W, int N,
                          int splits, AddendSlabs& left) {
    ddk_conv_args a = c.conv_args(kind, cw, src0, c0, src1, c1, out, H, W, N);
    a.bias = nullptr;
    a.defer_reduce = 1;
    const int s = kind == DDK_CONV3X3_S2 ? 2 : 1;
    left = AddendSlabs{splits, (long long)c.B * (H / s) * (W / s) * N, cw.has_bias ? c.P + cw.b : nullptr};
    return conv_forward(a, c.st);
}
static int run_conv_parts(Ctx& c, const ConvW& cw, const float* src0, int c0, const float* src1, int c1, float* raw, int H, int W, int N) {
    ddk_conv_args a = c.conv_args(DDK_CONV3X3_S1, cw, src0, c0, src1, c1, raw, H, W, N);
    a.gn_partials = c.W + c.ly.off_gn;
    a.gn_groups = GROUPS;
    return conv_forward(a, c.st);
}

enum ConvGnPath {
    CG_GENERIC,
    CG_LOCAL,
    CG_WLOCAL,
    CG_FIRST,
    CG_CLUSTER,
    CG_CLUSTER_SPLIT,
    CG_PARTS,
    CG_SLABS,
    CG_PLAIN
};
struct ConvGnChoice {
    ConvGnPath path = CG_PLAIN;
    int np = 0;
    int cl_splits = 1;
    int splits = 1;
    bool wino = false;
    bool local() const { return path == CG_LOCAL || path == CG_WLOCAL; }
};
static ConvGnChoice classify_conv_gn(const ddk_unet& u, const ConvW& cw, int B, int H, int W, int c0, int c1, int N, bool first_input,
                                     bool cluster, size_t splitk_floats) {
    ConvGnChoice k;
    const int cin = c0 + c1;
    auto is = [&](ConvGnPath p) { k.path = p; return k; };
    if (u.generic) return is(CG_GENERIC);
    if (cw.has_wl && (H * W == 16 || (H * W == 4 && B % 4 == 0)) && conv_gn_local_ok(H, W, cin, c0, N, GROUPS)) return is(CG_LOCAL);
    if (cw.has_wwl && H * W == 64 && conv_gn_wlocal_ok(H, W, cin, c0, N, GROUPS)) return is(CG_WLOCAL);
    k.wino = use_wino(cw, H, W, cin, N);
    if (cw.has_wf && first_input && conv_first_ok(u.cfg.in_ch, N, H, W, GROUPS)) return is(CG_FIRST);
    cluster = cluster && cw.has_wu && conv_wino_cluster_device_ok();
    k.np = cluster ? conv_wino_cluster_np(B, H, W, cin, N, GROUPS) : 0;
    if (k.np > 0 && k.np <= u.cluster_np_max) return is(CG_CLUSTER);
    k.np = cluster && u.cluster_split ? conv_wino_cluster_split_np(B, H, W, cin, N, GROUPS, &k.cl_splits) : 0;
    if (k.np > 0 && k.np <= u.cluster_np_max && (size_t)k.cl_splits * B * H * W * N <= splitk_floats &&
        conv_wino_cluster_pair_words(B, H, W, N) <= CL_PAIR_WORDS)
        return is(CG_CLUSTER_SPLIT);
    k.np = cw.has_wu ? conv_wino_stats_parts(B, H, W, cin, N, GROUPS) : 0;
    if (k.np > 0) return is(CG_PARTS);
    k.splits = k.wino ? conv_wino_splits(B, H, W, cin, N) : conv_splits(DDK_CONV3X3_S1, B, H, W, cin, N);
    return is(k.splits > 1 && groupnorm_workspace_bytes(B, H * W, N, GROUPS) == 0 ? CG_SLABS : CG_PLAIN);
}
static bool conv_gn_is_local(const ddk_unet& u, const ConvW& cw, int B, int H, int W, int c0, int c1, int N) {
    return classify_conv_gn(u, cw, B, H, W, c0, c1, N, false, false, 0).local();
}

static int run_conv_gn(Ctx& c, const ConvW& cw, const float* src0, int c0, const float* src1, int c1, float* raw, const NormW& n,
                       const float* temb, const float* addend, float* out, int H, int W, int N, const AddendSlabs& as = AddendSlabs(),
                       const AddendSlabs& ss = AddendSlabs()) {
    const ConvGnChoice k = classify_conv_gn(c.u, cw, c.B, H, W, c0, c1, N, c.x_first && src0 == c.x_padded && !src1,
                                            c.allow_cluster && c.n_cluster < c.u.cluster_limit, c.ly.splitk);
    if (ss.n > 1 && !k.local()) return fail_arg("run_conv_gn: slab source on a path that cannot sum it");
    if (as.n > 1 && !k.local())
        return fail_arg(k.path == CG_GENERIC ? "run_conv_gn: slab addend / source on the generic path"
                                             : "run_conv_gn: slab addend on a path that cannot sum it");
    const float* bias = cw.has_bias ? c.P + cw.b : nullptr;
    const float *g = c.P + n.g, *b = c.P + n.b;
    float* gnp = c.W + c.ly.off_gn;
    switch (k.path) {
        case CG_GENERIC:
            DDK_TRY(run_conv(c, DDK_CONV3X3_S1, cw, src0, c0, src1, c1, nullptr, raw, H, W, N));
            return groupnorm_mish_generic(raw, g, b, temb, c.u.temb_total, addend, out, c.B, H * W, N, n.c_real, GROUPS, GN_EPS, c.st, c.temb_rows);
        case CG_LOCAL:
        case CG_WLOCAL:
            return (k.path == CG_LOCAL ? conv_gn_local : conv_gn_wlocal)(src0, c0, src1, c1, c.P + (k.path == CG_LOCAL ? cw.wl : cw.wwl), bias, g, b,
                       temb, c.u.temb_total, c.temb_rows, addend, out, c.B, H, W, N, GROUPS, GN_EPS, c.st, as, ss);
        case CG_FIRST:
            DDK_TRY(conv_first(c.x_first, c.P + cw.wf, bias, raw, nullptr, c.B, H, W, c.u.cfg.in_ch, N, GROUPS, nullptr, nullptr, c.st));
            break;
        case CG_CLUSTER:
        case CG_CLUSTER_SPLIT: {
            ++c.n_cluster;
            ddk_conv_args a = c.conv_args(DDK_CONV3X3_S1, cw, src0, c0, src1, c1, out, H, W, N);
            a.resid = addend;
            WinoGnFuse f = c.gn_fuse(n, temb, c.temb_rows);
            if (k.path == CG_CLUSTER_SPLIT) f.pairs = reinterpret_cast<unsigned*>(c.W + c.ly.off_cl + cl_pair_offset(c.B));
            return conv_forward(a, c.st, nullptr, &f);
        }
        case CG_PARTS:
            DDK_TRY(run_conv_parts(c, cw, src0, c0, src1, c1, raw, H, W, N));
            return groupnorm_mish_parts(raw, gnp, k.np, g, b, temb, c.u.temb_total, addend, out, c.B, H * W, N, GROUPS, GN_EPS, c.st, c.temb_rows);
        case CG_SLABS: {
            AddendSlabs sl;
            DDK_TRY(run_conv_slabs(c, DDK_CONV3X3_S1, cw, src0, c0, src1, c1, raw, H, W, N, k.splits, sl));
            return groupnorm_mish_ex(c.W + c.ly.off_splitk, sl.n, sl.stride, sl.bias, g, b, temb, c.u.temb_total, addend, out, c.B, H * W, N,
                                     GROUPS, GN_EPS, nullptr, 0, c.st, c.temb_rows);
        }
        case CG_PLAIN:
            DDK_TRY(run_conv(c, DDK_CONV3X3_S1, cw, src0, c0, src1, c1, nullptr, raw, H, W, N));
            break;
    }
    return groupnorm_mish(raw, g, b, temb, c.u.temb_total, addend, out, c.B, H * W, N, GROUPS, GN_EPS, gnp, c.ly.gn_ws * sizeof(float), c.st,
                          c.temb_rows);
}

static bool res_takes_slab_source(const ddk_unet& u, const ResW& r, int B, int H, int W, int c0) {
    return !u.generic && !r.has_res && conv_gn_is_local(u, r.c1, B, H, W, c0, 0, r.co) && conv_gn_is_local(u, r.c2, B, H, W, r.co, 0, r.co);
}

static int run_res(Ctx& c, const ResW& r, const float* src0, int c0, const float* src1, int c1, float* out, int H, int W,
                   const AddendSlabs& ss = AddendSlabs()) {
    float* raw = c.W + c.ly.off_raw;
    float* a1 = c.W + c.ly.off_a1;
    float* res = c.W + c.ly.off_res;
    const float* addend = src0;
    AddendSlabs as;
    if (ss.n > 1) {
        if (r.has_res || src1) return fail_arg("run_res: slab source with a skip conv or a second source");
        as = ss;
    }
    if (r.has_res) {
        const int rs = conv_splits(DDK_CONV1X1, c.B, H, W, c0 + c1, r.co);
        if (rs > 1 && !conv1x1_sm_ok((long long)c.B * H * W, c0, c1, r.co) && conv_gn_is_local(c.u, r.c1, c.B, H, W, c0, c1, r.co) &&
            conv_gn_is_local(c.u, r.c2, c.B, H, W, r.co, 0, r.co)) {
            DDK_TRY(run_conv_slabs(c, DDK_CONV1X1, r.res, src0, c0, src1, c1, res, H, W, r.co, rs, as));
            addend = c.W + c.ly.off_splitk;
        } else {
            DDK_TRY(run_conv(c, DDK_CONV1X1, r.res, src0, c0, src1, c1, nullptr, res, H, W, r.co));
            addend = res;
        }
    }
    DDK_TRY(run_conv_gn(c, r.c1, src0, c0, src1, c1, raw, r.n1, c.temb + r.temb_off, nullptr, a1, H, W, r.co, AddendSlabs(), ss));
    return run_conv_gn(c, r.c2, a1, r.co, nullptr, 0, raw, r.n2, nullptr, addend, out, H, W, r.co, as);
}

static bool attn_fold_eligible(const ddk_unet& u, const AttnW& a, int B, int H, int W) {
    const long long M = (long long)B * H * W;
    return u.attn_fold && H * W > u.attn_fold_min_hw && (H * W) % 64 == 0 && attn_fold_ok(a.c, HEADS) && conv1x1_ws_ok(M, a.c, a.c) &&
           conv_ln_fold_ok(B, H, W, a.c, 2 * HIDDEN) && B <= 256;
}

static int run_attn(Ctx& c, const AttnW& a, const float* x, float* out, int H, int W) {
    float* xn = c.W + c.ly.off_xn;
    float* qkv = c.W + c.ly.off_qkv;
    float* ctx = c.W + c.ly.off_ctx;
    float* o = c.W + c.ly.off_o;
    const long long M = (long long)c.B * H * W;
    if (!c.u.generic && H * W <= 16 && a.c % 32 == 0 && linattn_small_qkv_ok(H * W, a.c)) {
        DDK_TRY(linattn_small_qkv(x, c.P + a.qkv_op, c.P + a.ln_c1, c.P + a.ln_c2, LN_EPS, ctx, o, c.B, H * W, a.c, HEADS, c.st));
        return run_conv(c, DDK_CONV1X1, a.out, o, HIDDEN, nullptr, 0, x, out, H, W, a.c);
    }
    if (!c.u.generic && attn_fold_eligible(c.u, a, c.B, H, W)) {
        if (c.u.attn_kvctx && attn_kvctx_ok(c.B, H * W, a.c, HEADS) && c.ly.splitk * sizeof(float) >= attn_kvctx_workspace_bytes(c.B, H * W)) {
            DDK_TRY(attn_kvctx(x, c.P + a.qkv_lnw + (size_t)HIDDEN * a.c, c.P + a.ln_c1 + HIDDEN, c.P + a.ln_c2 + HIDDEN, LN_EPS, ctx, c.B, H * W,
                               c.W + c.ly.off_splitk, c.ly.splitk * sizeof(float), c.st));
        } else {
            const ConvLnFold lnkv{c.P + a.ln_c1 + HIDDEN, c.P + a.ln_c2 + HIDDEN, LN_EPS};
            DDK_TRY(run_conv(c, DDK_CONV1X1, a.qkv, x, a.c, nullptr, 0, nullptr, qkv, H, W, 2 * HIDDEN, c.P + a.qkv_lnw + (size_t)HIDDEN * a.c,
                             &lnkv));
            DDK_TRY(linattn_context(qkv, ctx, c.B, H * W, HEADS, c.W + c.ly.off_splitk, c.ly.splitk * sizeof(float), c.st, true));
        }
        float* A = o;
        float* a1 = A + (size_t)c.B * a.c * a.c;
        float* a2 = a1 + (size_t)c.B * a.c;
        DDK_TRY(attn_fold(ctx, c.P + a.qkv_lnw, c.P + a.ln_c1, c.P + a.ln_c2, c.P + a.out.w, a.out.has_bias ? c.P + a.out.b : nullptr, A, a1,
                          a2, c.B, a.c, HEADS, c.st));
        const ConvLnFold lnA{a1, a2, LN_EPS};
        return conv1x1_ws(x, A, nullptr, x, out, M, a.c, &lnA, c.st, c.B);
// ... 844 lines not shown
```

### downsampled-diffusion_amd/ddk/lib.py

```python
import ctypes as C
import os

import torch

_HERE = os.path.dirname(os.path.abspath(__file__))
LIB_PATH = os.environ.get("DDK_LIB", os.path.join(os.path.dirname(_HERE), "csrc", "libddk.so"))


class DDKError(RuntimeError):
    pass


ABI_VERSION = 400
ERR_CLUSTER = -4


class ConvArgs(C.Structure):
    _fields_ = [
        ("kind", C.c_int), ("src0", C.c_void_p), ("src1", C.c_void_p), ("c0", C.c_int), ("c1", C.c_int),
        ("weight", C.c_void_p), ("bias", C.c_void_p), ("resid", C.c_void_p), ("out", C.c_void_p),
        ("B", C.c_int), ("H", C.c_int), ("W", C.c_int), ("N", C.c_int), ("pre_mish", C.c_int), ("post_mish", C.c_int), ("defer_reduce", C.c_int),
        ("workspace", C.c_void_p), ("workspace_bytes", C.c_size_t), ("weight_wino", C.c_void_p),
        ("gn_partials", C.c_void_p), ("gn_groups", C.c_int), ("mish_out", C.c_void_p), ("dmish_src", C.c_void_p),
    ]
# ... 57 lines not shown
    "ddk_pad_channels": (_I, [_P, _P, _LL, _I, _I, _P]),
    "ddk_pack_conv_weight": (_I, [_P, _P, _I, _I, _I, _I, _I, _P]),
    "ddk_pack_convT_weight": (_I, [_P, _P, _I, _I, _P]),
    "ddk_pack_conv_weight_split": (_I, [_P, _P, _I, _I, _I, _I, _I, _I, _I, _P]),
    "ddk_pack_convT_weight_padded": (_I, [_P, _P, _I, _I, _I, _P]),
    "ddk_pack_linear_T": (_I, [_P, _P, _I, _I, _I, _I, _P]),
    "ddk_pack_conv_weight_wino": (_I, [_P, _P, _I, _I, _I, _P]),
    "ddk_pack_conv_weight_wino_dgrad": (_I, [_P, _P, _I, _I, _I, _I, _I, _P]),
    "ddk_conv_wino_splits": (_I, [_I, _I, _I, _I, _I]),
    "ddk_pack_convT_weight_wino": (_I, [_P, _P, _I, _I, _I, _P]),
    "ddk_convT_wino_splits": (_I, [_I, _I, _I, _I, _I]),
    "ddk_conv_gn_partials": (_I, [_I, _I, _I, _I, _I, _I]),
    "ddk_groupnorm_mish_partials": (_I, [_P, _P, _I, _P, _P, _P, _I, _P, _P, _I, _I, _I, _I, _F, _P]),
    "ddk_pack_conv_weight_first": (_I, [_P, _P, _I, _I, _P]),
    "ddk_conv_first_ok": (_I, [_I, _I, _I, _I, _I]),
    "ddk_conv_first": (_I, [_P, _P, _P, _P, _P, _I, _I, _I, _I, _I, _I, _P]),
    "ddk_conv1x1_ws_ok": (_I, [C.c_longlong, _I, _I]),
    "ddk_conv1x1_ws": (_I, [_P, _P, _P, _P, _P, C.c_longlong, _I, _P, _P, _F, _P]),
    "ddk_conv1x1_ws_images": (_I, [_P, _P, _P, _P, _P, C.c_longlong, _I, _P, _P, _F, _I, _P]),
    "ddk_linattn_context_kv": (_I, [_P, _P, _I, _I, _I, _P, _SZ, _P]),
    "ddk_attention_fold": (_I, [_P, _P, _P, _P, _P, _P, _P, _P, _P, _I, _I, _I, _P]),
    "ddk_groupnorm_mish_partials_res1x1": (_I, [_P, _P, _I, _P, _P, _P, _I, _P, _P, _P, _I, _P, _I, _I, _I, _I, _F, _P]),
    "ddk_final_tail": (_I, [_P, _P, _I, _P, _P, _F, _P, _P, _I, _P, _P, _P, _P, _P, _P, _P, _P, _P, C.c_uint64, C.c_uint32, _I, _I, _I, _I, _P]),
    "ddk_pack_conv_weight_local": (_I, [_P, _P, _I, _I, _I, _P]),
    "ddk_pack_conv1x1_weight_local": (_I, [_P, _P, _I, _I, _I, _P]),
    "ddk_pack_convT_weight_local": (_I, [_P, _P, _I, _I, _P]),
    "ddk_pack_conv_weight_wino_local": (_I, [_P, _P, _I, _I, _I, _P]),
    "ddk_conv3x3_gn_mish_wino_ok": (_I, [_I, _I, _I, _I, _I, _I]),
    "ddk_conv3x3_gn_mish_wino": (_I, [_P, _I, _P, _I, _P, _P, _P, _P, _P, _I, _P, _P, _I, _I, _I, _I, _I, _F, _P]),
    "ddk_conv3x3_gn_mish_slabs": (_I, [_P, _I, _LL, _P, _I, _P, _P, _P, _P, _P, _I, _P, _I, _LL, _P, _P, _I, _I, _I, _I, _I, _F, _P]),
    "ddk_attention_kv_context_workspace_bytes": (_SZ, [_I, _I]),
    "ddk_attention_kv_context_ok": (_I, [_I, _I, _I, _I]),
    "ddk_attention_kv_context": (_I, [_P, _P, _P, _P, _F, _P, _I, _I, _P, _SZ, _P]),
    "ddk_pack_qkv_operand": (_I, [_P, _P, _I, _I, _P]),
    "ddk_linattn_small_from_x": (_I, [_P, _P, _P, _P, _F, _P, _P, _I, _I, _I, _I, _P]),
    "ddk_conv3x3_gn_mish_ok": (_I, [_I, _I, _I, _I, _I, _I]),
    "ddk_conv3x3_gn_mish": (_I, [_P, _I, _P, _I, _P, _P, _P, _P, _P, _I, _P, _P, _I, _I, _I, _I, _I, _F, _P]),
    "ddk_conv_workspace_bytes": (_SZ, [_I, _I, _I, _I, _I, _I]),
    "ddk_conv_splits": (_I, [_I, _I, _I, _I, _I, _I]),
    "ddk_conv_forward": (_I, [C.POINTER(ConvArgs), _P]),
    "ddk_debug_read_stamps": (_I, [_P]),
    "ddk_groupnorm_mish": (_I, [_P, _P, _P, _P, _I, _P, _P, _I, _I, _I, _I, _F, _P, _SZ, _P]),
    "ddk_groupnorm_workspace_bytes": (_SZ, [_I, _I, _I, _I]),
    "ddk_groupnorm_mish_slabs": (_I, [_P, _I, _LL, _P, _P, _P, _P, _I, _P, _P, _I, _I, _I, _I, _F, _P]),
    "ddk_chan_layernorm": (_I, [_P, _P, _P, _P, _LL, _I, _F, _P]),
    "ddk_mish": (_I, [_P, _P, _LL, _P]),
    "ddk_tanh": (_I, [_P, _P, _LL, _P]),
    "ddk_avgpool2": (_I, [_P, _P, _I, _I, _I, _I, _P]),
    "ddk_upsample_nearest2": (_I, [_P, _P, _I, _I, _I, _I, _P]),
    "ddk_add": (_I, [_P, _P, _P, _LL, _P]),
    "ddk_linattn_context_workspace_bytes": (_SZ, [_I, _I, _I]),
    "ddk_linattn_context": (_I, [_P, _P, _I, _I, _I, _P, _SZ, _P]),
    "ddk_linattn_apply": (_I, [_P, _P, _P, _I, _I, _I, _P]),
    "ddk_linattn_fused_small": (_I, [_P, _P, _P, _I, _I, _I, _P]),
    "ddk_time_mlp": (_I, [_P, _P, _P, _P, _P, _P, _P, _P, _I, _I, _P]),
    "ddk_time_proj": (_I, [_P, _P, _P, _P, _I, _I, _I, _P]),
    "ddk_conv1x1_small_n": (_I, [_P, _P, _P, _P, _LL, _I, _I, _P]),
    "ddk_q_sample": (_I, [_P, _P, _P, _P, _P, _P, _I, _LL, _P]),
    "ddk_p_sample_update": (_I, [_P, _P, _P, _P, _P, _P, _P, _P, _P, _I, _LL, C.c_uint64, C.c_uint32, _P]),
    "ddk_p_sample_update_multistep": (_I, [_P, _P, _P, _P, _P, _P, _P, _P, _P, _I, _LL, _P]),
    "ddk_p_sample_update_inpaint": (_I, [_P] * 14 + [_I, _LL, C.c_uint64, C.c_uint32, _P]),
    "ddk_p_sample_update_restore": (_I, [_P, _P, _P, _I] + [_P] * 6 + [_I, _I, _I, _I, C.c_uint64, C.c_uint32, _P]),
    "ddk_randn": (_I, [_P, _LL, C.c_uint64, C.c_uint32, C.c_uint32, _P]),
    "ddk_fix_samples": (_I, [_P, _P, _I, _I, _I, _I, _P]),
    "ddk_sq_err_sum": (_I, [_P, _P, _P, _I, _LL, _P]),
    "ddk_vlb_terms_workspace_bytes": (_SZ, [_I, _LL]),
    "ddk_vlb_terms": (_I, [_P, _P, _P, _P, _P, _P, _P, _P, _P, _P, _P, _P, _I, _LL, _P, _SZ, _P]),
    "ddk_unet_create": (_P, [C.POINTER(UnetConfig)]),
    "ddk_unet_destroy": (None, [_P]),
    "ddk_unet_num_slots": (_I, [_P]),
    "ddk_unet_slot_name": (C.c_char_p, [_P, _I]),
    "ddk_unet_slot_numel": (_LL, [_P, _I]),
    "ddk_unet_packed_bytes": (_SZ, [_P]),
    "ddk_unet_pack_slot": (_I, [_P, _I, _P, _P, _P]),
    "ddk_unet_finalize_pack": (_I, [_P, _P, _P]),
    "ddk_unet_workspace_bytes": (_SZ, [_P, _I, _I, _I]),
    "ddk_unet_forward": (_I, [_P, _P, _P, _P, _P, _I, _I, _I, _P, _SZ, _P]),
    "ddk_conv3x3_gn_mish_cluster_ok": (_I, [_I, _I, _I, _I, _I, _I]),
    "ddk_conv3x3_gn_mish_cluster_workspace_bytes": (_SZ, [_I, _I, _I, _I]),
    "ddk_conv3x3_gn_mish_cluster_split_workspace_bytes": (_SZ, [_I, _I, _I, _I, _I, _I]),
    "ddk_conv3x3_gn_mish_cluster": (_I, [_P, _I, _P, _I, _P, _P, _P, _P, _P, _I, _P, _P, _I, _I, _I, _I, _I, _F, _P, _SZ, _P]),
    "ddk_unet_set_option": (_I, [_P, _I, _I]),
    "ddk_debug_cluster_timeouts": (C.c_uint, []),
    "ddk_conv3x3_gn_mish_cluster_check": (_I, [_P, _I, _P]),
    "ddk_unet_cluster_check": (_I, [_P, _P, _I, _I, _I, _P]),
    "ddk_debug_occupy": (_I, [_I, _I, _I, _P]),
    "ddk_debug_clock_probe": (_I, [_P, _I, _P]),
    "ddk_unet_flops": (C.c_double, [_P, _I, _I, _I]),
    "ddk_unet_flops_executed": (C.c_double, [_P, _I, _I, _I]),
    "ddk_sampler_workspace_bytes": (_SZ, [_P, _I, _I, _I, _I]),
    "ddk_sampler_run": (_I, [C.POINTER(SamplerArgs), _P]),
    "ddk_sampler_run_spaced": (_I, [C.POINTER(SamplerArgs), C.POINTER(C.c_int64), _P]),
    "ddk_sampler_multistep_workspace_bytes": (_SZ, [_P, _I, _I, _I, _I]),
    "ddk_sampler_run_multistep": (_I, [C.POINTER(SamplerArgs), C.POINTER(C.c_int64), _P, _P]),
    "ddk_sampler_inpaint_workspace_bytes": (_SZ, [_P, _I, _I, _I, _I]),
    "ddk_sampler_run_inpaint": (_I, [C.POINTER(SamplerArgs), C.POINTER(InpaintArgs), _P]),
    "ddk_sampler_restore_workspace_bytes": (_SZ, [_P, _I, _I, _I, _I]),
    "ddk_sampler_restore_tail_parts": (_I, [_P, _I, _I, _I, _I]),
    "ddk_sampler_run_restore": (_I, [C.POINTER(SamplerArgs), C.POINTER(C.c_int64), _P, _I, _P]),
    "ddk_sampler_invalidate": (_I, [_P]),
    "ddk_sampler_release_workspace": (_I, [_P, _P]),
    "ddk_vlb_sweep_workspace_bytes": (_SZ, [_P, _I, _I, _I, _I]),
    "ddk_vlb_sweep_run": (_I, [C.POINTER(VlbSweepArgs), _P]),
    "ddk_pack_conv_weight_dgrad": (_I, [_P, _P, _I, _I, _I, _I, _I, _I, _P]),
    "ddk_zero_stuff2": (_I, [_P, _P, _I, _I, _I, _I, _I, _I, _P]),
    "ddk_conv_wgrad_workspace_bytes": (_SZ, [_I, _I, _I, _I, _I, _I]),
    "ddk_conv_wgrad": (_I, [_I, _P, _P, _P, _I, _I, _I, _I, _I, _I, _I, _I, _P, _SZ, _P]),
    "ddk_conv_wgrad_bias": (_I, [_I, _P, _P, _P, _P, _I, _I, _I, _I, _I, _I, _I, _I, _P, _SZ, _P]),
    "ddk_bias_grad": (_I, [_P, _P, _LL, _I, _I, _P, _SZ, _P]),
    "ddk_groupnorm_train_workspace_bytes": (_SZ, [_I, _I, _I, _I]),
    "ddk_dropout_epoch": (_I, [C.c_uint64, _I, _P]),
    "ddk_groupnorm_mish_train_fwd": (_I, [_P, _P, _P, _P, _I, _P, _F, C.c_uint64, C.c_uint32, _P, _I, _I, _I, _I, _F, _P, _SZ, _P]),
    "ddk_groupnorm_mish_bwd": (_I, [_P, _P, _P, _F, C.c_uint64, C.c_uint32, _P, _P, _P, _I, _I, _I, _I, _F, _P, _SZ, _P]),
    "ddk_groupnorm_mish_train_fwd_slabs": (_I, [_P, _I, _LL, _P, _P, _P, _P, _P, _I, _P, _F, C.c_uint64, C.c_uint32, _P, _I, _I, _I, _I,
                                                _F, _P]),
    "ddk_groupnorm_mish_bwd_slabs": (_I, [_P, _P, _P, _F, C.c_uint64, C.c_uint32, _P, _I, _LL, _P, _P, _I, _I, _I, _I, _F, _P]),
    "ddk_rows_sum": (_I, [_P, _I, _LL, _P, _I, _I, _P]),
    "ddk_rows_sum_batched": (_I, [_P, _I, _LL, _I, _LL, _P, _I, _I, _P]),
    "ddk_rows_sum_targets": (_I, [_P, _I, _LL, _I, _LL, _P, _P, _P, _P, _I, _I, _P]),
    "ddk_multi_add": (_I, [_P, _P, _I, _LL, _P]),
    "ddk_conv_wgrad_defer": (_I, [_I, _P, _P, _P, _P, _I, _I, _I, _I, _I, _I, _I, _I, _P, _SZ, _P, _P]),
    "ddk_wgrad_reduce_jobs": (_I, [_P, _I, _P]),
    "ddk_rows_sum_jobs": (_I, [_P, _I, _P]),
    "ddk_pack_jobs_layout": (_LL, [_P, _I]),
    "ddk_pack_jobs": (_I, [_P, _I, _LL, _P]),
    "ddk_chan_layernorm_bwd": (_I, [_P, _P, _P, _P, _P, _I, C.POINTER(C.c_int), _LL, _I, _F, _P]),
    "ddk_chan_layernorm_bwd_add": (_I, [_P, _P, _P, _P, _P, _P, _I, C.POINTER(C.c_int), _LL, _I, _F, _P]),
    "ddk_groupnorm_mish_generic_train_fwd": (_I, [_P, _P, _P, _P, _I, _P, _F, C.c_uint64, C.c_uint32, _P, _I, _I, _I, _I, _I, _F, _P]),
    "ddk_groupnorm_mish_generic_bwd": (_I, [_P, _P, _P, _F, C.c_uint64, C.c_uint32, _P, _P, _P, _I, _I, _I, _I, _I, _F, _P]),
    "ddk_chan_layernorm_generic": (_I, [_P, _P, _P, _P, _LL, _I, _I, _F, _P]),
    "ddk_chan_layernorm_generic_bwd": (_I, [_P, _P, _P, _P, _P, _P, _I, C.POINTER(C.c_int), _LL, _I, _I, _F, _P]),
    "ddk_linattn_train_workspace_bytes": (_SZ, [_I, _I, _I]),
    "ddk_linattn_stats": (_I, [_P, _P, _I, _I, _I, _P, _SZ, _P]),
    "ddk_linattn_bwd": (_I, [_P, _P, _P, _P, _P, _P, _I, _I, _I, _P, _SZ, _P]),
    "ddk_linattn_bwd_recompute": (_I, [_P, _P, _P, _P, _P, _P, _I, _I, _I, _P, _SZ, _P]),
    "ddk_mish_bwd": (_I, [_P, _P, _P, _LL, _P]),
    "ddk_tanh_bwd": (_I, [_P, _P, _P, _LL, _P]),
    "ddk_avgpool2_bwd": (_I, [_P, _P, _I, _I, _I, _I, _P]),
    "ddk_upsample_nearest2_bwd": (_I, [_P, _P, _I, _I, _I, _I, _P]),
    "ddk_sq_err_grad": (_I, [_P, _P, _P, _P, _I, _LL, _P]),
    "ddk_ae_objective": (_I, [_P, _P, _P, _I, _I, _P, _P]),
    "ddk_ae_objective_bwd": (_I, [_P, _P, _I, _I, _P, _P, _P]),
    "ddk_scale_per_sample": (_I, [_P, _P, _P, _I, _LL, _P]),
    "ddk_conv1x1_small_n_bwd": (_I, [_P, _P, _P, _P, _P, _I, C.POINTER(C.c_int), _LL, _I, _I, _P]),
    "ddk_small_gemm_workspace_bytes": (_SZ, [_I, _I, _I, _I]),
    "ddk_small_gemm": (_I, [_I, _P, _P, _P, _I, _I, _I, _I, _I, _I, _I, _P, _SZ, _P]),
    "ddk_sincos_embed": (_I, [_P, _P, _P, _I, _I, _P]),
    "ddk_bias_act": (_I, [_P, _P, _P, _LL, _I, _P]),
    "ddk_grad_norm_clip": (_I, [_P, _LL, _F, _P, _P, _SZ, _P]),
    "ddk_adam_step": (_I, [_P, _P, _P, _P, _LL, C.c_double, C.c_double, C.c_double, C.c_double, _I, _P, _P]),
    "ddk_ema_update": (_I, [_P, _P, _LL, _F, _P]),
}

_lib = None


def load():
    global _lib
    if _lib is not None:
        return _lib
    if not os.path.exists(LIB_PATH):
        raise DDKError(
            f"HIP kernel library not found at {LIB_PATH}. Build it with `make -C {os.path.dirname(LIB_PATH)}` "
            "(or `python -c 'import __graft_entry__ as g; g.build()'`). There is no CPU fallback.")
    lib = C.CDLL(LIB_PATH)
    for name, (res, args) in SIGNATURES.items():
# ... 32 lines not shown
```

### include/ddk.h

```cpp
#ifndef DDK_H
#define DDK_H

#include <stddef.h>
#include <stdint.h>

#ifdef __cplusplus
extern "C" {
#endif

typedef void* ddk_stream_t;

#define DDK_OK 0
#define DDK_ERR_ARG (-1)
#define DDK_ERR_HIP (-2)
#define DDK_ERR_WORKSPACE (-3)
#define DDK_ERR_CLUSTER (-4)

int ddk_version(void);
const char* ddk_last_error(void);
int ddk_device_ok(void);

int ddk_nchw_to_nhwc(const float* src, float* dst, int B, int C, int H, int W, int c_pad, ddk_stream_t s);
int ddk_nhwc_to_nchw(const float* src, float* dst, int B, int C, int H, int W, int c_stride, ddk_stream_t s);
int ddk_pad_channels(const float* src, float* dst, long long M, int C, int c_pad, ddk_stream_t s);
// ... 100 lines not shown

size_t ddk_linattn_context_workspace_bytes(int B, int HW, int heads);
int ddk_linattn_context(const float* qkv, float* ctx, int B, int HW, int heads, void* workspace, size_t workspace_bytes, ddk_stream_t s);
int ddk_linattn_context_kv(const float* kv, float* ctx, int B, int HW, int heads, void* workspace, size_t workspace_bytes, ddk_stream_t s);
int ddk_attention_fold(const float* ctx, const float* wqg, const float* c1q, const float* c2q, const float* wout, const float* bout, float* A,
                       float* a1, float* a2, int B, int C, int heads, ddk_stream_t s);
size_t ddk_attention_kv_context_workspace_bytes(int B, int HW);
int ddk_attention_kv_context_ok(int B, int HW, int C, int heads);
int ddk_attention_kv_context(const float* x, const float* w_kv, const float* c1, const float* c2, float ln_eps, float* ctx, int B, int HW,
                             void* workspace, size_t workspace_bytes, ddk_stream_t s);
int ddk_linattn_fused_small(const float* qkv, float* ctx, float* out, int B, int HW, int heads, ddk_stream_t s);
int ddk_linattn_apply(const float* qkv, const float* ctx, float* out, int B, int HW, int heads, ddk_stream_t s);
int ddk_pack_qkv_operand(const float* folded_w, float* dst, int heads, int c_pad, ddk_stream_t s);
int ddk_linattn_small_from_x(const float* x, const float* w_operand, const float* c1, const float* c2, float ln_eps, float* ctx,
                             float* out, int B, int HW, int C, int heads, ddk_stream_t s);

int ddk_time_mlp(const int64_t* t, const float* freqs, const float* w1t, const float* b1, const float* w2t,
                 const float* b2, float* act, float* raw, int B, int dim, ddk_stream_t s);
int ddk_time_proj(const float* act, const float* wt, const float* bias, float* out, int B, int dim, int n_out,
                  ddk_stream_t s);

int ddk_conv1x1_small_n(const float* x, const float* w, const float* bias, float* out, long long M, int C,
                        int n_out, ddk_stream_t s);

int ddk_q_sample(const float* x, const float* eps, const int64_t* t, const float* sqrt_acp,
                 const float* sqrt_1m_acp, float* out, int B, long long per, ddk_stream_t s);
int ddk_p_sample_update(float* x, const float* eps_hat, const float* noise, const int64_t* t,
                        const float* c_recip, const float* c_recipm1, const float* c1, const float* c2,
                        const float* sigma, int B, long long per, uint64_t seed, uint32_t stream_id,
                        ddk_stream_t s);
int ddk_p_sample_update_multistep(float* x, const float* eps_hat, float* x0_hist, const int64_t* t, const float* c_recip,
                                  const float* c_recipm1, const float* c1, const float* c2, const float* c3, int B, long long per,
                                  ddk_stream_t s);
int ddk_p_sample_update_inpaint(float* x, const float* eps_hat, const float* known, const float* mask, const int64_t* t,
                                const float* c_recip, const float* c_recipm1, const float* c1, const float* c2, const float* sigma,
                                const float* ka, const float* kb, const float* ja, const float* jb, int B, long long per, uint64_t seed,
                                uint32_t stream_id, ddk_stream_t s);
int ddk_p_sample_update_restore(float* x, const float* eps_hat, const float* y, int n, const int64_t* t, const float* c_recip,
                                const float* c_recipm1, const float* c1, const float* c2, const float* sigma, int B, int H, int W,
                                int channels, uint64_t seed, uint32_t stream_id, ddk_stream_t s);
int ddk_final_tail(const float* raw, const float* partials, int tiles_per_image, const float* gamma, const float* beta, float eps,
                   const float* w, const float* bias, int n_out, float* eps_out, float* x, const float* noise, const int64_t* t,
                   const float* c_recip, const float* c_recipm1, const float* c1, const float* c2, const float* sigma, uint64_t seed,
                   uint32_t stream_id, int B, int HW, int C, int groups, ddk_stream_t s);
int ddk_randn(float* out, long long n, uint64_t seed, uint32_t step, uint32_t stream_id, ddk_stream_t s);
int ddk_fix_samples(const float* x_nchw, float* out_nhwc, int B, int C, int H, int W, ddk_stream_t s);
size_t ddk_vlb_terms_workspace_bytes(int B, long long per);
int ddk_vlb_terms(const float* x, const float* x_t, const float* eps_hat, const float* eps, const int64_t* t,
                  const float* c_recip, const float* c_recipm1, const float* c1, const float* c2,
                  const float* post_logvar, float* vlb, float* sqerr, int B, long long per, void* workspace,
                  size_t workspace_bytes, ddk_stream_t s);
int ddk_sq_err_sum(const float* a, const float* b, float* per_sample, int B, long long per, ddk_stream_t s);

typedef struct ddk_unet_config {
    int in_ch;
    int chan;
    int n_levels;
    int mults[8];
} ddk_unet_config;

typedef struct ddk_unet ddk_unet;

ddk_unet* ddk_unet_create(const ddk_unet_config* cfg);
void ddk_unet_destroy(ddk_unet* u);
int ddk_unet_num_slots(const ddk_unet* u);
const char* ddk_unet_slot_name(const ddk_unet* u, int slot);
long long ddk_unet_slot_numel(const ddk_unet* u, int slot);
size_t ddk_unet_packed_bytes(const ddk_unet* u);
int ddk_unet_pack_slot(const ddk_unet* u, int slot, const float* canonical, void* packed, ddk_stream_t s);
int ddk_unet_finalize_pack(const ddk_unet* u, void* packed, ddk_stream_t s);
size_t ddk_unet_workspace_bytes(const ddk_unet* u, int B, int H, int W);
int ddk_unet_forward(const ddk_unet* u, const void* packed, const float* x, const int64_t* t, float* out,
                     int B, int H, int W, void* workspace, size_t workspace_bytes, ddk_stream_t s);
#define DDK_OPT_CLUSTER_GROUPNORM 1
#define DDK_OPT_ATTENTION_FOLD 3
#define DDK_OPT_FOLD_DOWNSAMPLE_REDUCE 5
#define DDK_OPT_ATTENTION_KV_CONTEXT 6
#define DDK_OPT_LEVEL_CHAIN 7
#define DDK_OPT_FIRST_GROUPNORM 8
#define DDK_OPT_RESTORE_FUSED_TAIL 12
int ddk_unet_set_option(ddk_unet* u, int option, int value);
int ddk_unet_cluster_check(const ddk_unet* u, void* workspace, int B, int H, int W, ddk_stream_t s);
unsigned ddk_debug_cluster_timeouts(void);
int ddk_debug_clock_probe(unsigned long long* out, int workgroups, ddk_stream_t s);
int ddk_debug_occupy(int workgroups, int lds_bytes, int microseconds, ddk_stream_t s);
double ddk_unet_flops(const ddk_unet* u, int B, int H, int W);
double ddk_unet_flops_executed(const ddk_unet* u, int B, int H, int W);

typedef struct ddk_sampler_args {
    const ddk_unet* unet;
    const void* packed;
    float* x;
    const float* noise;
    const float* c_recip;
    const float* c_recipm1;
    const float* c1;
    const float* c2;
    const float* sigma;
    int B, H, W;
    int t_start;
    int t_end;
    uint64_t seed;
    uint32_t stream_id;
    int use_graph;
    void* workspace;
    size_t workspace_bytes;
} ddk_sampler_args;

size_t ddk_sampler_workspace_bytes(const ddk_unet* u, int B, int H, int W, int t_start);
int ddk_sampler_run(const ddk_sampler_args* a, ddk_stream_t s);
int ddk_sampler_run_spaced(const ddk_sampler_args* a, const int64_t* timestep_map, ddk_stream_t s);
size_t ddk_sampler_multistep_workspace_bytes(const ddk_unet* u, int B, int H, int W, int t_start);
int ddk_sampler_run_multistep(const ddk_sampler_args* a, const int64_t* timestep_map, const float* c3, ddk_stream_t s);
typedef struct ddk_inpaint_args {
    const int64_t* timestep_map;
    const float* known;
    const float* mask;
    const float* ka;
    const float* kb;
    const float* ja;
    const float* jb;
} ddk_inpaint_args;
size_t ddk_sampler_inpaint_workspace_bytes(const ddk_unet* u, int B, int H, int W, int n_ops);
int ddk_sampler_run_inpaint(const ddk_sampler_args* a, const ddk_inpaint_args* ip, ddk_stream_t s);
size_t ddk_sampler_restore_workspace_bytes(const ddk_unet* u, int B, int H, int W, int t_start);
int ddk_sampler_restore_tail_parts(const ddk_unet* u, int B, int H, int W, int n);
int ddk_sampler_run_restore(const ddk_sampler_args* a, const int64_t* timestep_map, const float* y, int n, ddk_stream_t s);
int ddk_sampler_invalidate(ddk_unet* u);
int ddk_sampler_release_workspace(ddk_unet* u, const void* workspace);

typedef struct ddk_vlb_sweep_args {
    const ddk_unet* unet;
    const void* packed;
    const float* x;
    const float* noise;
    const float* sqrt_acp;
    const float* sqrt_1m_acp;
    const float* c_recip;
    const float* c_recipm1;
    const float* c1;
    const float* c2;
    const float* post_logvar;
    int B, H, W;
    int T;
    uint64_t seed;
    uint32_t stream_id;
    int use_graph;
    void* workspace;
    size_t workspace_bytes;
    float* vlb_t;
    float* l_simple_t;
} ddk_vlb_sweep_args;

size_t ddk_vlb_sweep_workspace_bytes(const ddk_unet* u, int B, int H, int W, int T);
int ddk_vlb_sweep_run(const ddk_vlb_sweep_args* a, ddk_stream_t s);



int ddk_pack_conv_weight_wino_dgrad(const float* w_oihw, float* dst, int O, int I, int c_lo, int c_hi, int o_pad, ddk_stream_t s);
int ddk_pack_convT_weight_wino(const float* w_iohw, float* dst, int I, int O, int i_pad, ddk_stream_t s);
int ddk_convT_wino_splits(int B, int H, int W, int cin, int N);
int ddk_pack_conv_weight_dgrad(const float* w_oihw, float* dst, int O, int I, int KH, int KW, int i_pad, int o_pad,
                               ddk_stream_t s);
int ddk_zero_stuff2(const float* in, float* out, int B, int H, int W, int Ho, int Wo, int C, ddk_stream_t s);
size_t ddk_conv_wgrad_workspace_bytes(int kind, int B, int H, int W, int cx, int N);
int ddk_conv_wgrad(int kind, const float* x, const float* dy, float* grad_w, int B, int H, int W, int cx, int c_real,
// ... 112 lines not shown
```

Baseline: 25.99.

## Add unsplit cluster Winograd tile splitting K across waves inside one workgroup

```diff
diff --git a/downsampled-diffusion_amd/csrc/conv_igemm.hip b/downsampled-diffusion_amd/csrc/conv_igemm.hip
--- a/downsampled-diffusion_amd/csrc/conv_igemm.hip
+++ b/downsampled-diffusion_amd/csrc/conv_igemm.hip
@@ -1199,7 +1199,7 @@
     if (a.weight_wino && !a.pre_mish && !act_epilogue && conv_wino_ok(a.kind, a.H, a.W, a.c0 + a.c1, a.N)) {
         DDK_REQUIRE(aligned16(a.weight_wino), "conv: weight_wino alignment");
         DDK_TRY(ensure_device_init());
-        const int ws = conv_wino_splits(a.B, a.H, a.W, a.c0 + a.c1, a.N);
+        const int ws = fuse && fuse->unsplit ? 1 : conv_wino_splits(a.B, a.H, a.W, a.c0 + a.c1, a.N);
         const long long slab = (long long)a.B * a.H * a.W * a.N;
         if (ws > 1) {
             const size_t need = (size_t)(fuse ? ws - 1 : ws) * slab * sizeof(float);
diff --git a/downsampled-diffusion_amd/csrc/conv_wino.hip b/downsampled-diffusion_amd/csrc/conv_wino.hip
--- a/downsampled-diffusion_amd/csrc/conv_wino.hip
+++ b/downsampled-diffusion_amd/csrc/conv_wino.hip
@@ -589,6 +589,8 @@
                                 (int)(W2<4>::LDS_FL * sizeof(float))));
     DDK_HIP(hipFuncSetAttribute(reinterpret_cast<const void*>(&conv3x3_wino2_kernel<4, 0, true>), hipFuncAttributeMaxDynamicSharedMemorySize,
                                 (int)(W2<4>::LDS_FL * sizeof(float))));
+    DDK_HIP(hipFuncSetAttribute(reinterpret_cast<const void*>(&conv3x3_wino2_kernel<8, 0, true>), hipFuncAttributeMaxDynamicSharedMemorySize,
+                                (int)(W2<8>::LDS_FL * sizeof(float))));
 #ifdef DDK_TUNING
 #define W2_DBG_ATTR(P_, D_) DDK_HIP(hipFuncSetAttribute(reinterpret_cast<const void*>(&conv3x3_wino2_kernel<P_, D_, false>), \
                                                 hipFuncAttributeMaxDynamicSharedMemorySize, (int)(W2<P_>::LDS_FL * sizeof(float))))
@@ -631,11 +633,25 @@
     if (mt * nt * splits > 256) return 0;
     return np;
 }
+constexpr int W2K_MAX_CIN = 128;
+static std::atomic<int> g_wino_unsplit{1};
+int conv_wino_set_unsplit(int level) { return g_wino_unsplit.exchange(level < 0 ? 0 : level > 2 ? 2 : level, std::memory_order_relaxed); }
+int conv_wino_unsplit_level() { return g_wino_unsplit.load(std::memory_order_relaxed); }
+int conv_wino_cluster_unsplit_np(int B, int H, int W, int cin, int N, int groups, int level) {
+    if (level <= 0 || (level == 1 && cin > W2K_MAX_CIN) || !conv_wino_ok(DDK_CONV3X3_S1, H, W, cin, N) || groups <= 0 || N % groups) return 0;
+    if (conv_wino_splits(B, H, W, cin, N) <= 1) return 0;
+    constexpr int nt_w = W2<8>::NT;
+    const int cpg = N / groups, tpi = (H / 2) * (W / 2);
+    if (N % nt_w || cpg % 4 || cpg > nt_w || nt_w % cpg || tpi % WBT) return 0;
+    const int np = tpi / WBT;
+    if (np > 8 || N / nt_w > 8 || (long long)B * np * (N / nt_w) > 256) return 0;
+    return np;
+}
 size_t conv_wino_cluster_pair_words(int B, int H, int W, int N) {
     return (size_t)ceil_div((long long)B * (H / 2) * (W / 2), WBT) * (size_t)(N / WBN) * 16;
 }
 size_t conv_wino_cluster_ws_floats(int B, int H, int W, int N) {
-    const long long mt = (long long)B * (H / 2) * (W / 2) / WBT, nt = N / WBN;
+    const long long mt = (long long)B * (H / 2) * (W / 2) / WBT, nt = N / W2<8>::NT;
     return (size_t)(mt * nt * 32 + (long long)B * nt * 16);
 }
 
@@ -660,9 +676,12 @@
 
 int conv_wino_forward(const ddk_conv_args& a, int splits, hipStream_t st, const WinoGnFuse* fuse) {
     WinoParams p{};
+    const bool unsplit = fuse && fuse->unsplit;
     if (fuse) {
-        const int np = splits == 1 ? conv_wino_cluster_np(a.B, a.H, a.W, a.c0 + a.c1, a.N, fuse->groups)
-                                   : conv_wino_cluster_split_np(a.B, a.H, a.W, a.c0 + a.c1, a.N, fuse->groups, nullptr);
+        DDK_REQUIRE(!unsplit || (splits == 1 && !fuse->res_x), "conv(wino, cluster): the unsplit tile takes one split and no 1x1 addend");
+        const int np = unsplit       ? conv_wino_cluster_unsplit_np(a.B, a.H, a.W, a.c0 + a.c1, a.N, fuse->groups, 2)
+                       : splits == 1 ? conv_wino_cluster_np(a.B, a.H, a.W, a.c0 + a.c1, a.N, fuse->groups)
+                                     : conv_wino_cluster_split_np(a.B, a.H, a.W, a.c0 + a.c1, a.N, fuse->groups, nullptr);
         DDK_REQUIRE(np > 0 && !a.post_mish && !a.gn_partials, "conv(wino): shape not eligible for the in-launch GroupNorm");
         if (splits > 1) {
             DDK_REQUIRE(fuse->pairs && a.workspace && aligned16(a.workspace) && !fuse->res_x,
@@ -705,6 +724,11 @@
     p.dTW = make_fastdiv_u((unsigned)p.TW);
     p.dTH = make_fastdiv_u((unsigned)p.TH);
     if (p.splits > 1 && !fuse) p.out = static_cast<float*>(a.workspace);
+    if (unsplit) {
+        dim3 grid8((unsigned)(p.tiles / WBT), (unsigned)(a.N / W2<8>::NT), 1u);
+        hipLaunchKernelGGL((conv3x3_wino2_kernel<8, 0, true>), grid8, dim3(768), (size_t)W2<8>::LDS_FL * sizeof(float), st, p);
+        return check_launch("conv3x3_wino2_kernel<cluster, unsplit>");
+    }
     const int variant = wino_variant(a.B, a.H, a.W, a.N);
     if (variant != WINO_V_OLD) {
         dim3 grid2((unsigned)ceil_div(p.tiles, WBT), (unsigned)(a.N / wino_nt(variant)), (unsigned)p.splits);
@@ -839,7 +863,14 @@
 extern "C" int ddk_conv3x3_gn_mish_cluster_ok(int B, int H, int W, int cin, int N, int groups) {
     if (!ddk::conv_wino_cluster_device_ok()) return 0;
     const int np = ddk::conv_wino_cluster_np(B, H, W, cin, N, groups);
-    return np > 0 ? np : ddk::conv_wino_cluster_split_np(B, H, W, cin, N, groups, nullptr);
+    if (np > 0) return np;
+    const int nu = ddk::conv_wino_cluster_unsplit_np(B, H, W, cin, N, groups, ddk::conv_wino_unsplit_level());
+    return nu > 0 ? nu : ddk::conv_wino_cluster_split_np(B, H, W, cin, N, groups, nullptr);
+}
+extern "C" int ddk_debug_set_wino_unsplit(int level) { return ddk::conv_wino_set_unsplit(level); }
+extern "C" int ddk_debug_wino_unsplit_taken(int B, int H, int W, int cin, int N, int groups) {
+    return ddk::conv_wino_cluster_device_ok() && ddk::conv_wino_cluster_np(B, H, W, cin, N, groups) <= 0 &&
+           ddk::conv_wino_cluster_unsplit_np(B, H, W, cin, N, groups, ddk::conv_wino_unsplit_level()) > 0;
 }
 extern "C" size_t ddk_conv3x3_gn_mish_cluster_workspace_bytes(int B, int H, int W, int N) {
     if (B <= 0 || H <= 0 || W <= 0 || N <= 0 || N % ddk::WBN) return 0;
@@ -877,7 +908,8 @@
     DDK_REQUIRE(conv_wino_cluster_device_ok() && ddk_conv3x3_gn_mish_cluster_ok(B, H, W, c0 + c1, N, groups) > 0,
                 "conv3x3_gn_mish_cluster: shape or device not eligible (ddk_conv3x3_gn_mish_cluster_ok)");
     const size_t plain_bytes = ddk_conv3x3_gn_mish_cluster_workspace_bytes(B, H, W, N);
-    const size_t split_bytes = ddk_conv3x3_gn_mish_cluster_split_workspace_bytes(B, H, W, c0 + c1, N, groups);
+    const bool unsplit = ddk_debug_wino_unsplit_taken(B, H, W, c0 + c1, N, groups) != 0;
+    const size_t split_bytes = unsplit ? 0 : ddk_conv3x3_gn_mish_cluster_split_workspace_bytes(B, H, W, c0 + c1, N, groups);
     DDK_REQUIRE(workspace_bytes >= (split_bytes ? split_bytes : plain_bytes) && aligned16(workspace), "conv3x3_gn_mish_cluster: workspace");
     float* ws = static_cast<float*>(workspace);
     DDK_HIP(hipMemsetAsync(ws, 0, cl_front_floats(B) * sizeof(float), as_stream(s)));
@@ -894,6 +926,7 @@
     a.B = B; a.H = H; a.W = W; a.N = N;
     const ClWords w = cl_words(ws, B);
     WinoGnFuse f{gamma, beta, temb, nullptr, temb_stride, eps, groups, ws + cl_front_floats(B), w.counters, w.fail};
+    f.unsplit = unsplit;
     if (split_bytes) {
         f.pairs = reinterpret_cast<unsigned*>(pairs);
         a.workspace = pairs + conv_wino_cluster_pair_words(B, H, W, N);
diff --git a/downsampled-diffusion_amd/csrc/conv_wino2_kernel.inc b/downsampled-diffusion_amd/csrc/conv_wino2_kernel.inc
--- a/downsampled-diffusion_amd/csrc/conv_wino2_kernel.inc
+++ b/downsampled-diffusion_amd/csrc/conv_wino2_kernel.inc
@@ -12,22 +12,26 @@
 #endif
 template <int P>
 struct W2 {
-    static constexpr int NT = 256 / P;
+    static constexpr bool KH = P == 8;
+    static constexpr int PS = KH ? 4 : P;
+    static constexpr int NT = KH ? 32 : 256 / P;
     static constexpr int NB = NT / 32;
-    static constexpr int SPC = 16 / P;
-    static constexpr int SPR = 4 / P;
-    static constexpr int V_FL = P * WBT * 32;
-    static constexpr int U_FL = P * NT * 32;
+    static constexpr int SPC = 16 / PS;
+    static constexpr int SPR = 4 / PS;
+    static constexpr int V_FL = PS * WBT * 32;
+    static constexpr int U_FL = PS * NT * 32;
     static constexpr int STAGE = V_FL + U_FL;
     static constexpr int PPI = NT / 8;
+    static constexpr int NPIECE = PS * PPI;
     static constexpr int TP = NT + 4;
-    static constexpr int T_FL = 4 * 2 * WBT * TP;
+    static constexpr int NBLK = KH ? 8 : 4;
+    static constexpr int T_FL = NBLK * 2 * WBT * TP;
     static constexpr int LDS_FL = (3 * STAGE > T_FL + 320) ? 3 * STAGE : T_FL + 320;
     static constexpr int QUADS = NT / 4;
     static constexpr int ITEMS = 2 * WBT * QUADS / 512;
-    static constexpr int LPL = P == 2 ? DDK_WINO2_LP_F : DDK_WINO2_LP_D;
-    static constexpr int LPM = (32 - 4 * LPL) / 8;
-    static_assert(4 * LPL + 8 * LPM == 32 && LPL % 2 == 0 && LPM % 2 == 0, "piece split: (8,0), (4,2) or (0,4)");
+    static constexpr int LPL = KH ? 4 : P == 2 ? DDK_WINO2_LP_F : DDK_WINO2_LP_D;
+    static constexpr int LPM = (NPIECE - 4 * LPL) / 8;
+    static_assert(4 * LPL + 8 * LPM == NPIECE && LPL % 2 == 0 && LPM % 2 == 0, "piece split: (8,0), (4,2) or (0,4); K (4,0)");
 };
 #ifndef DDK_WINO2_STAGGER
 #define DDK_WINO2_STAGGER 1
@@ -39,7 +43,8 @@
 template <int P, int DBG, bool CL>
 __global__ __launch_bounds__(768) void conv3x3_wino2_kernel(const WinoParams p) {
     using G = W2<P>;
-    constexpr int NT = G::NT, SPC = G::SPC, SPR = G::SPR, STAGE = G::STAGE, V_FL = G::V_FL;
+    constexpr int NT = G::NT, SPC = G::SPC, SPR = G::SPR, STAGE = G::STAGE, V_FL = G::V_FL, PS = G::PS;
+    constexpr bool KH = G::KH;
     extern __shared__ __attribute__((aligned(16))) float smem[];
     unsigned long long r_entry = 0;
     if (DBG) r_entry = __builtin_amdgcn_s_memrealtime();
@@ -66,7 +71,7 @@
     const unsigned uv_odd = (unsigned)((prow * 32 + ((ppos ^ (4 + (prow >> 1))) << 2)) * 4);
     auto issue_u = [&](int T, int buf, int g_first, auto count) {
         const int chunk = c_begin + T / SPC, st = T % SPC;
-        const float* base = p.wu + (((long long)chunk * 16 + P * st) * p.N + n0) * 32;
+        const float* base = p.wu + (((long long)chunk * 16 + PS * st) * p.N + n0) * 32;
         const unsigned dst = lds_base + (unsigned)((buf * STAGE + V_FL) * 4);
 #pragma unroll
         for (int j = 0; j < decltype(count)::value; ++j) {
@@ -141,7 +146,7 @@
             using I0 = std::integral_constant<int, 0>; using I1 = std::integral_constant<int, 1>;
             using I2 = std::integral_constant<int, 2>; using I3 = std::integral_constant<int, 3>;
             float* base = smem + buf * STAGE + v_off;
-            if constexpr (P == 4) {
+            if constexpr (PS == 4) {
                 const f32x4 r0 = rowc(I0{}), r1 = rowc(I1{}), r2 = rowc(I2{}), r3 = rowc(I3{});
                 *reinterpret_cast<f32x4*>(base + 0 * (WBT * 32)) = r0 - r2;
                 *reinterpret_cast<f32x4*>(base + 1 * (WBT * 32)) = r1 + r2;
@@ -170,23 +175,23 @@
         };
         load_row(c_begin, 0);
         load_row(c_begin, 2);
-        if (P == 4) load_row(c_begin, 1);
+        if (PS == 4) load_row(c_begin, 1);
         if (!(DBG & 2)) issue_u(0, 0, lw * G::LPL, std::integral_constant<int, G::LPL>{});
-        if (P == 2) load_row(c_begin, 1);
+        if (PS == 2) load_row(c_begin, 1);
         constexpr int NPL0 = (DBG & 2) ? 0 : G::LPL;
-        wait_vmcnt<NPL0 + (P == 2 ? 4 : 0)>();
+        wait_vmcnt<NPL0 + (PS == 2 ? 4 : 0)>();
         pin();
         using K0 = std::integral_constant<int, 0>;
         if (!(DBG & 8)) {
             write_v(K0{}, K0{}, 0);
-            if (P == 2) write_v(K0{}, std::integral_constant<int, SPR - 1>{}, 1);
+            if (PS == 2) write_v(K0{}, std::integral_constant<int, SPR - 1>{}, 1);
             else write_v(std::integral_constant<int, 1 / SPR>{}, K0{}, 1);
             if (1 < n_chunks) load_row(c_begin + 1, 0);
-            if (P == 4) load_row(c_begin, 3);
+            if (PS == 4) load_row(c_begin, 3);
         }
         if (!(DBG & 2)) issue_u(1, 1, lw * G::LPL, std::integral_constant<int, G::LPL>{});
         if (DBG & 8) wait_vmcnt<NPL0>();
-        else if (P == 2) { if (1 < n_chunks) wait_vmcnt<NPL0 + 8>(); else wait_vmcnt<NPL0 + 4>(); }
+        else if (PS == 2) { if (1 < n_chunks) wait_vmcnt<NPL0 + 8>(); else wait_vmcnt<NPL0 + 4>(); }
         else { if (1 < n_chunks) wait_vmcnt<NPL0 + 8>(); else wait_vmcnt<NPL0 + 4>(); }
         asm volatile("s_waitcnt lgkmcnt(0)" ::: "memory");
         __builtin_amdgcn_s_barrier();
@@ -223,7 +228,7 @@
         return;
     }
 
-    const int pp = wid % P, nb = wid / P;
+    const int pp = wid % PS, nb = KH ? 0 : wid / PS, kh = KH ? wid / PS : 0;
     f32x16 acc[SPC];
 #pragma unroll
     for (int i = 0; i < SPC; ++i)
@@ -320,7 +325,54 @@
             }
             if (STG) mma4(acc[SPC - 1], a[0], b[0]);
         };
-        if (W2_STAGGER && wid >= 4) mloop(std::true_type{}); else mloop(std::false_type{});
+        auto mloop_k = [&](auto stgc) {
+            constexpr bool STG = decltype(stgc)::value;
+            float4 a[2], b[2];
+            int buf = 0;
+            const int fa = (lane & 31) * 32 + (((4 * kh + fh) ^ fsw) << 2), fb = (lane & 31) * 32 + (((4 * kh + 2 + fh) ^ fsw) << 2);
+            auto mma4 = [&](f32x16& c, const float4& av, const float4& bv) {
+                c = __builtin_amdgcn_mfma_f32_32x32x2f32(av.x, bv.x, c, 0, 0, 0);
+                c = __builtin_amdgcn_mfma_f32_32x32x2f32(av.y, bv.y, c, 0, 0, 0);
+                c = __builtin_amdgcn_mfma_f32_32x32x2f32(av.z, bv.z, c, 0, 0, 0);
+                c = __builtin_amdgcn_mfma_f32_32x32x2f32(av.w, bv.w, c, 0, 0, 0);
+            };
+            if (!STG) a[0] = *reinterpret_cast<const float4*>(smem + a_img + fa);
+            for (int c = 0; c < n_chunks; ++c) {
+                static_for<SPC>([&](auto sc) {
+                    constexpr int s = decltype(sc)::value;
+                    const float* As = smem + buf * STAGE + a_img;
+                    const float* Bs = smem + buf * STAGE + b_img;
+                    const int nbuf = buf == 2 ? 0 : buf + 1;
+                    if constexpr (!STG) {
+                        b[0] = *reinterpret_cast<const float4*>(Bs + fa);
+                        a[1] = *reinterpret_cast<const float4*>(As + fb);
+                        b[1] = *reinterpret_cast<const float4*>(Bs + fb);
+                        __builtin_amdgcn_sched_barrier(0);
+                        mma4(acc[s], a[0], b[0]);
+                        a[0] = *reinterpret_cast<const float4*>(smem + nbuf * STAGE + a_img + fa);
+                        __builtin_amdgcn_sched_barrier(0);
+                        mma4(acc[s], a[1], b[1]);
+                    } else {
+                        a[1] = *reinterpret_cast<const float4*>(As + fa);
+                        b[1] = *reinterpret_cast<const float4*>(Bs + fa);
+                        if (s > 0 || c > 0) {
+                            __builtin_amdgcn_sched_barrier(0);
+                            mma4(acc[(s + SPC - 1) % SPC], a[0], b[0]);
+                        }
+                        a[0] = *reinterpret_cast<const float4*>(As + fb);
+                        b[0] = *reinterpret_cast<const float4*>(Bs + fb);
+                        __builtin_amdgcn_sched_barrier(0);
+                        mma4(acc[s], a[1], b[1]);
+                    }
+                    asm volatile("s_waitcnt lgkmcnt(0)" ::: "memory");
+                    __builtin_amdgcn_s_barrier();
+                    buf = nbuf;
+                });
+            }
+            if (STG) mma4(acc[SPC - 1], a[0], b[0]);
+        };
+        if constexpr (KH) { if (W2_STAGGER && wid >= 4) mloop_k(std::true_type{}); else mloop_k(std::false_type{}); }
+        else if (W2_STAGGER && wid >= 4) mloop(std::true_type{}); else mloop(std::false_type{});
         if (DBG && lane == 0 && wid == 0) {
             const int wg = (blockIdx.x + gridDim.x * (blockIdx.y + gridDim.y * blockIdx.z)) & 1023;
             unsigned long long tE;
@@ -339,8 +391,8 @@
         for (int r = 0; r < 16; ++r) {
             const int row = (r & 3) + 8 * (r >> 2) + 4 * (lane >> 5);
             const int col = nb * 32 + (lane & 31);
-            if constexpr (P == 4) {
-                float* Ts = smem + pp * (2 * WBT * TP);
+            if constexpr (PS == 4) {
+                float* Ts = smem + (kh * 4 + pp) * (2 * WBT * TP);
                 const float m0 = acc[0][r], m1 = acc[1][r], m2 = acc[2][r], m3 = acc[3][r];
                 Ts[row * TP + col] = (m0 + m1) + m2;
                 Ts[(WBT + row) * TP + col] = (m1 - m2) - m3;
@@ -388,9 +440,17 @@
         const float4 q2 = *reinterpret_cast<const float4*>(tp + 2 * (2 * WBT * TP));
         const float4 q3 = *reinterpret_cast<const float4*>(tp + 3 * (2 * WBT * TP));
         float4 y0, y1;
-        if constexpr (P == 4) {
+        if constexpr (PS == 4) {
             y0 = f4add(f4add(q0, q1), q2);
             y1 = f4sub(f4sub(q1, q2), q3);
+            if constexpr (KH) {
+                const float4 r0 = *reinterpret_cast<const float4*>(tp + 4 * (2 * WBT * TP));
+                const float4 r1 = *reinterpret_cast<const float4*>(tp + 5 * (2 * WBT * TP));
+                const float4 r2 = *reinterpret_cast<const float4*>(tp + 6 * (2 * WBT * TP));
+                const float4 r3 = *reinterpret_cast<const float4*>(tp + 7 * (2 * WBT * TP));
+                y0 = f4add(y0, f4add(f4add(r0, r1), r2));
+                y1 = f4add(y1, f4sub(f4sub(r1, r2), r3));
+            }
         } else {
             y0 = f4add(q0, q2);
             y1 = f4add(q1, q3);
@@ -427,7 +487,7 @@
         keep[it][0] = y0;
         keep[it][1] = y1;
     }
-    if (CLS && p.splits > 1) {
+    if constexpr (CLS) if (p.splits > 1) {
         unsigned* pair = p.cl_pair + ((long long)tile_m * gridDim.y + tile_n) * 16;
         if (partner) {
             asm volatile("s_waitcnt vmcnt(0)" ::: "memory");
diff --git a/downsampled-diffusion_amd/csrc/ddk_internal.h b/downsampled-diffusion_amd/csrc/ddk_internal.h
--- a/downsampled-diffusion_amd/csrc/ddk_internal.h
+++ b/downsampled-diffusion_amd/csrc/ddk_internal.h
@@ -130,6 +130,7 @@
     float* records;
     unsigned* counters;
     unsigned* fail;
+    bool unsplit = false;
     unsigned* pairs = nullptr;
     const float* res_x = nullptr;
     const float* res_w = nullptr;
@@ -144,6 +145,9 @@
 int conv_wino_forward(const ddk_conv_args& a, int splits, hipStream_t st, const WinoGnFuse* fuse = nullptr);
 int conv_wino_cluster_np(int B, int H, int W, int cin, int N, int groups);
 int conv_wino_cluster_split_np(int B, int H, int W, int cin, int N, int groups, int* splits_out);
+int conv_wino_cluster_unsplit_np(int B, int H, int W, int cin, int N, int groups, int level);
+int conv_wino_set_unsplit(int level);
+int conv_wino_unsplit_level();
 size_t conv_wino_cluster_pair_words(int B, int H, int W, int N);
 bool conv_wino_variant_new(int B, int H, int W, int N);
 bool conv_wino_cluster_device_ok();
diff --git a/downsampled-diffusion_amd/csrc/unet_plan.hip b/downsampled-diffusion_amd/csrc/unet_plan.hip
--- a/downsampled-diffusion_amd/csrc/unet_plan.hip
+++ b/downsampled-diffusion_amd/csrc/unet_plan.hip
@@ -113,6 +113,7 @@
     bool first_gn = true;
     int level_chain = 9;
     int level_chain_max_batch = 32;
+    int cluster_unsplit = 1;
     int attn_fold_min_hw = 256;
     bool attn_fold = true;
     bool generic = false;
@@ -416,6 +417,7 @@
         {2, false, [](ddk_unet& p, int v) { p.cluster_limit = v; }},
         {4, true, [](ddk_unet& p, int v) { p.cluster_np_max = v; }},
         {11, true, [](ddk_unet& p, int v) { p.cluster_split = v != 0; }},
+        {13, true, [](ddk_unet& p, int v) { p.cluster_unsplit = v < 0 ? 0 : v > 2 ? 2 : v; }},
     };
     for (const auto& o : options) {
         if (o.option != option) continue;
@@ -717,6 +719,7 @@
     CG_WLOCAL,
     CG_FIRST,
     CG_CLUSTER,
+    CG_CLUSTER_UNSPLIT,
     CG_CLUSTER_SPLIT,
     CG_PARTS,
     CG_SLABS,
@@ -744,6 +747,8 @@
     k.np = cluster ? conv_wino_cluster_np(B, H, W, cin, N, GROUPS) : 0;
     if (k.np > 0 && k.np <= u.cluster_np_max) return is(CG_CLUSTER);
     k.np = cluster && u.cluster_split ? conv_wino_cluster_split_np(B, H, W, cin, N, GROUPS, &k.cl_splits) : 0;
+    if (k.np > 0 && k.np <= u.cluster_np_max && conv_wino_cluster_unsplit_np(B, H, W, cin, N, GROUPS, u.cluster_unsplit) == k.np)
+        return is(CG_CLUSTER_UNSPLIT);
     if (k.np > 0 && k.np <= u.cluster_np_max && (size_t)k.cl_splits * B * H * W * N <= splitk_floats &&
         conv_wino_cluster_pair_words(B, H, W, N) <= CL_PAIR_WORDS)
         return is(CG_CLUSTER_SPLIT);
@@ -780,11 +785,13 @@
             DDK_TRY(conv_first(c.x_first, c.P + cw.wf, bias, raw, nullptr, c.B, H, W, c.u.cfg.in_ch, N, GROUPS, nullptr, nullptr, c.st));
             break;
         case CG_CLUSTER:
+        case CG_CLUSTER_UNSPLIT:
         case CG_CLUSTER_SPLIT: {
             ++c.n_cluster;
             ddk_conv_args a = c.conv_args(DDK_CONV3X3_S1, cw, src0, c0, src1, c1, out, H, W, N);
             a.resid = addend;
             WinoGnFuse f = c.gn_fuse(n, temb, c.temb_rows);
+            f.unsplit = k.path == CG_CLUSTER_UNSPLIT;
             if (k.path == CG_CLUSTER_SPLIT) f.pairs = reinterpret_cast<unsigned*>(c.W + c.ly.off_cl + cl_pair_offset(c.B));
             return conv_forward(a, c.st, nullptr, &f);
         }
diff --git a/downsampled-diffusion_amd/ddk/lib.py b/downsampled-diffusion_amd/ddk/lib.py
--- a/downsampled-diffusion_amd/ddk/lib.py
+++ b/downsampled-diffusion_amd/ddk/lib.py
@@ -163,6 +163,8 @@
     "ddk_conv3x3_gn_mish_cluster": (_I, [_P, _I, _P, _I, _P, _P, _P, _P, _P, _I, _P, _P, _I, _I, _I, _I, _I, _F, _P, _SZ, _P]),
     "ddk_unet_set_option": (_I, [_P, _I, _I]),
     "ddk_debug_cluster_timeouts": (C.c_uint, []),
+    "ddk_debug_set_wino_unsplit": (_I, [_I]),
+    "ddk_debug_wino_unsplit_taken": (_I, [_I, _I, _I, _I, _I, _I]),
     "ddk_conv3x3_gn_mish_cluster_check": (_I, [_P, _I, _P]),
     "ddk_unet_cluster_check": (_I, [_P, _P, _I, _I, _I, _P]),
     "ddk_debug_occupy": (_I, [_I, _I, _I, _P]),
diff --git a/include/ddk.h b/include/ddk.h
--- a/include/ddk.h
+++ b/include/ddk.h
@@ -206,6 +206,8 @@
 int ddk_unet_set_option(ddk_unet* u, int option, int value);
 int ddk_unet_cluster_check(const ddk_unet* u, void* workspace, int B, int H, int W, ddk_stream_t s);
 unsigned ddk_debug_cluster_timeouts(void);
+int ddk_debug_set_wino_unsplit(int level);
+int ddk_debug_wino_unsplit_taken(int B, int H, int W, int cin, int N, int groups);
 int ddk_debug_clock_probe(unsigned long long* out, int workgroups, ddk_stream_t s);
 int ddk_debug_occupy(int workgroups, int lds_bytes, int microseconds, ddk_stream_t s);
 double ddk_unet_flops(const ddk_unet* u, int B, int H, int W);
```

New measurement: 26.20, median of 6. About the same (+0.8%).
